# singhhp1069/charon

Measured on AMD Instinct MI355X. Metric: verified+aggregated 3-of-4 threshold BLS sigs/sec at 1/2/4/8 MI355X, higher is better.
Workload: dtype u32 (Fp 14x28-bit limbs); 1 GPU; config2: 3-of-4, 10000 DVs x 1 attestation per GPU; parallelism=shard1, inflight_launches=3, batches_per_launch=16, rlc_group=16, rlc_chunk=8, gident=0, subgroup_batch=0, level0=passed, hw_queues=4

## Files before the change

### charon_amd/csrc/bls_pair.h

```cpp
#pragma once
#include "bls_lines.h"

namespace tbg {

TBG_HD Fp pair_mul_lane(uint32_t par, const Fp& a, const Fp& ap, const Fp& b, const Fp& bp) {
  const Fp nbp = fp_neg_l(bp);
  return fp_mul2(a, fp_select(par != 0, bp, b), ap, fp_select(par != 0, b, nbp));
}
TBG_HD Fp pair_sqr_lane(uint32_t par, const Fp& a, const Fp& ap) {
  const Fp x = fp_add_l(fp_select(par != 0, ap, a), ap);
  const Fp y = fp_select(par != 0, a, fp_sub_l(a, ap));
  return fp_mul(x, y);
}
TBG_HD Fp pair_conj_lane(uint32_t par, const Fp& a) { return fp_select(par != 0, fp_neg(a), a); }
TBG_HD Fp pair_mul_xi_lane(uint32_t par, const Fp& a, const Fp& ap) {
  return fp_select(par != 0, fp_add(a, ap), fp_sub(a, ap));
}
TBG_HD Fp pair_inv_lane(uint32_t par, const Fp& a, const Fp& ap) {
  const Fp t = fp_inv(fp_mul2(a, a, ap, ap));
  return fp_mul(pair_conj_lane(par, a), t);
}
TBG_HD Fp pair_const(uint32_t par, const Fp2Const& c) { return par ? fp_from_const(c.c1) : fp_from_const(c.c0); }

struct Fp2p { Fp c0, c1; };
TBG_HD Fp2p f_add(const Fp2p& a, const Fp2p& b) { return {fp_add(a.c0, b.c0), fp_add(a.c1, b.c1)}; }
TBG_HD Fp2p f_sub(const Fp2p& a, const Fp2p& b) { return {fp_sub(a.c0, b.c0), fp_sub(a.c1, b.c1)}; }
TBG_HD Fp2p f_add_l(const Fp2p& a, const Fp2p& b) { return {fp_add_l(a.c0, b.c0), fp_add_l(a.c1, b.c1)}; }
TBG_HD Fp2p f_sub_l(const Fp2p& a, const Fp2p& b) { return {fp_sub_l(a.c0, b.c0), fp_sub_l(a.c1, b.c1)}; }
TBG_HD Fp2p f_neg(const Fp2p& a) { return {fp_neg(a.c0), fp_neg(a.c1)}; }
TBG_HD Fp2p f_reduce(const Fp2p& a) { return {fp_reduce(a.c0), fp_reduce(a.c1)}; }
TBG_HD Fp2p f_small(const Fp2p& a, uint32_t k) { return {fp_mul_small(a.c0, k), fp_mul_small(a.c1, k)}; }
TBG_HD Fp2p f_mul(const Fp2p& a, const Fp2p& b) {
  return {pair_mul_lane(0, a.c0, a.c1, b.c0, b.c1), pair_mul_lane(1, a.c1, a.c0, b.c1, b.c0)};
}
TBG_HD Fp2p f_sqr(const Fp2p& a) { return {pair_sqr_lane(0, a.c0, a.c1), pair_sqr_lane(1, a.c1, a.c0)}; }
TBG_HD Fp2p f_inv(const Fp2p& a) { return {pair_inv_lane(0, a.c0, a.c1), pair_inv_lane(1, a.c1, a.c0)}; }
TBG_HD bool f_is_zero(const Fp2p& a) { return fp_is_zero(a.c0) && fp_is_zero(a.c1); }
TBG_HD bool f_eq(const Fp2p& a, const Fp2p& b) { return fp_eq(a.c0, b.c0) && fp_eq(a.c1, b.c1); }
TBG_HD Fp2p pp_conj(const Fp2p& a) { return {pair_conj_lane(0, a.c0), pair_conj_lane(1, a.c1)}; }
TBG_HD Fp2p pp_mul_xi(const Fp2p& a) { return {pair_mul_xi_lane(0, a.c0, a.c1), pair_mul_xi_lane(1, a.c1, a.c0)}; }
TBG_HD Fp2p pp_mul_const(const Fp2p& a, const Fp2Const& c) {
  return {pair_mul_lane(0, a.c0, a.c1, pair_const(0, c), pair_const(1, c)),
          pair_mul_lane(1, a.c1, a.c0, pair_const(1, c), pair_const(0, c))};
}
TBG_HD Fp2p rlc_mul_c(const Fp2p& a, const Fp& c) { return {fp_mul(a.c0, c), fp_mul(a.c1, c)}; }
TBG_HD Fp2p f_conj(const Fp2p& a) { return pp_conj(a); }
TBG_HD Fp2p f_mulc(const Fp2p& a, const Fp2Const& c) { return pp_mul_const(a, c); }
template <> TBG_HD Fp2p f_zero<Fp2p>() { return {fp_zero(), fp_zero()}; }
template <> TBG_HD Fp2p f_one<Fp2p>() { return {fp_one(), fp_zero()}; }
TBG_HD Fp2p pp_from(const Fp2& a) { return {a.c0, a.c1}; }
TBG_HD Fp2 pp_to(const Fp2p& a) { return {a.c0, a.c1}; }

template <class F>
TBG_HD Jac<F> g2_psi_g(const Jac<F>& p) {
  return {f_mulc(f_conj(p.X), PSI_X), f_mulc(f_conj(p.Y), PSI_Y), f_reduce(f_conj(p.Z))};
}

template <class F>
TBG_HD Jac<F> jac_add_x(const Jac<F>& p, const Jac<F>& q, bool& exc) {
  if (jac_is_inf(p)) return q;
  if (jac_is_inf(q)) return p;
  const F Z1Z1 = f_sqr(p.Z);
  const F Z2Z2 = f_sqr(q.Z);
  const F S1 = f_mul(f_mul(p.Y, q.Z), Z2Z2);
  const F S2 = f_mul(f_mul(q.Y, p.Z), Z1Z1);
  const F Zs = f_reduce(f_sub_l(f_sqr(f_add(p.Z, q.Z)), f_add(Z1Z1, Z2Z2)));
  const F U1 = f_mul(p.X, Z2Z2);
  const F H = f_reduce(f_sub_l(f_mul(q.X, Z1Z1), U1));
  const F Rr = f_reduce(f_sub_l(S2, S1));
  if (f_is_zero(H)) {
    if (f_is_zero(Rr)) exc = true;
    return jac_inf<F>();
  }
  const F Z3 = f_mul(Zs, H);
  const F H2 = f_add(H, H);
  const F I = f_sqr(H2);
  const F J = f_mul(H, I);
  const F V = f_mul(U1, I);
  const F r2 = f_add(Rr, Rr);
  const F X3 = f_reduce(f_sub_l(f_sub_l(f_sqr(r2), J), f_add(V, V)));
  const F Y3 = f_reduce(f_sub_l(f_mul(f_sub_l(V, X3), r2), f_small(f_mul(S1, J), 2)));
  return {X3, Y3, Z3};
}

template <class F>
TBG_HD Jac<F> jac_dbl_lo(const Jac<F>& p) {
  const F YZ = f_mul(p.Y, p.Z);
  const F Z3 = f_reduce(f_add_l(YZ, YZ));
  const F B = f_sqr(p.Y);
  const F A = f_sqr(p.X);
  const F C = f_sqr(B);
  const F t = f_sub_l(f_sqr(f_add(p.X, B)), f_add(A, C));
  const F D = f_reduce(f_add_l(t, t));
  const F E = f_small(A, 3);
  const F X3 = f_reduce(f_sub_l(f_sqr(E), f_add(D, D)));
  const F Y3 = f_reduce(f_sub_l(f_mul(f_sub_l(D, X3), E), f_small(C, 8)));
  return {X3, Y3, Z3};
}

template <class F>
TBG_HD Jac<F> jac_add_aff_x(const Jac<F>& p, const Aff<F>& q, bool& exc) {
  if (jac_is_inf(p)) return jac_from_aff(q);
  F Z1Z1 = f_sqr(p.Z);
  F U2 = f_mul(q.x, Z1Z1);
  F S2 = f_mul(f_mul(q.y, p.Z), Z1Z1);
  F H = f_reduce(f_sub_l(U2, p.X));
  F Rr = f_reduce(f_sub_l(S2, p.Y));
  if (f_is_zero(H)) {
    if (f_is_zero(Rr)) exc = true;
    return jac_inf<F>();
  }
  F HH = f_sqr(H);
  F I = f_small(HH, 4);
  F J = f_mul(H, I);
  F r2 = f_add(Rr, Rr);
  F V = f_mul(p.X, I);
  F X3 = f_reduce(f_sub_l(f_sub_l(f_sqr(r2), J), f_add(V, V)));
  F Y3 = f_reduce(f_sub_l(f_mul(f_sub_l(V, X3), r2), f_small(f_mul(p.Y, J), 2)));
  F Z3 = f_reduce(f_sub_l(f_sub_l(f_sqr(f_add(p.Z, H)), Z1Z1), HH));
  return {X3, Y3, Z3};
}

template <class F>
TBG_HD Jac<F> jac_mul_xabs_aff_x(const Aff<F>& p, bool& exc) {
  Jac<F> acc = jac_from_aff(p);
#pragma unroll 1
  for (int i = 62; i >= 0; --i) {
    acc = jac_dbl_lo(acc);
    if ((X_ABS >> i) & 1) acc = jac_add_aff_x(acc, p, exc);
  }
  return acc;
}

template <class F>
TBG_HD Jac<F> jac_mul_xabs_x(const Jac<F>& p, bool& exc) {
  Jac<F> acc = p;
#pragma unroll 1
  for (int i = 62; i >= 0; --i) {
    acc = jac_dbl_lo(acc);
    if ((X_ABS >> i) & 1) acc = jac_add_x(acc, p, exc);
  }
  return acc;
}

template <class F>
TBG_HD Jac<F> g2_clear_cofactor_g(const Jac<F>& p, bool& exc) {
  const Jac<F> a = jac_neg(jac_mul_xabs_x(p, exc));
  const Jac<F> pp = g2_psi_g(p);
  const Jac<F> b = jac_add_x(a, pp, exc);
  Jac<F> u = g2_psi_g(g2_psi_g(jac_dbl_lo(p)));
  u = jac_add_x(u, jac_neg(pp), exc);
  u = jac_add_x(u, jac_neg(a), exc);
  u = jac_add_x(u, jac_neg(p), exc);
  const Jac<F> c = jac_neg(jac_mul_xabs_x(b, exc));
  return jac_add_x(u, c, exc);
}

template <class F> struct LineG { F l0, l1, l4; };

template <class F, bool EVAL = true, class S>
TBG_HD void miller_dbl_s(Jac<F>& T, const Fp& nxP, const Fp& yP, S&& sink) {
  const F ZZ = f_sqr(T.Z);
  const F YZ = f_mul(T.Y, T.Z);
  const F Z3 = f_reduce(f_add_l(YZ, YZ));
  const F l4 = f_mul(Z3, ZZ);
  sink(2, EVAL ? f_mulfp(l4, yP) : l4);
  const F B = f_sqr(T.Y);
  const F C = f_sqr(B);
  const F A = f_sqr(T.X);
  const F t = f_sub_l(f_sqr(f_add(T.X, B)), f_add(A, C));
  const F D = f_reduce(f_add_l(t, t));
  const F E = f_small(A, 3);
  const F l1 = f_mul(ZZ, E);
  sink(1, EVAL ? f_mulfp(l1, nxP) : l1);
  sink(0, f_reduce(f_sub_l(f_mul(T.X, E), f_add(B, B))));
  const F X3 = f_reduce(f_sub_l(f_sqr(E), f_add(D, D)));
  const F Y3 = f_reduce(f_sub_l(f_mul(f_sub_l(D, X3), E), f_small(C, 8)));
  T = {X3, Y3, Z3};
}

template <class F, bool EVAL = true, class S>
TBG_HD void miller_add_s(Jac<F>& T, const Aff<F>& Q, const Fp& nxP, const Fp& yP, S&& sink) {
  const F ZZ = f_sqr(T.Z);
  const F U2 = f_mul(Q.x, ZZ);
  const F S2 = f_mul(f_mul(Q.y, T.Z), ZZ);
  const F H = f_reduce(f_sub_l(U2, T.X));
  const F R = f_reduce(f_sub_l(S2, T.Y));
  const F Z3 = f_mul(T.Z, H);
  sink(2, EVAL ? f_mulfp(Z3, yP) : Z3);
  sink(1, EVAL ? f_mulfp(R, nxP) : R);
  sink(0, f_reduce(f_sub_l(f_mul(R, Q.x), f_mul(Q.y, Z3))));
  const F HH = f_sqr(H);
  const F HHH = f_mul(H, HH);
  const F V = f_mul(T.X, HH);
  const F X3 = f_reduce(f_sub_l(f_sub_l(f_sqr(R), HHH), f_add(V, V)));
  const F Y3 = f_reduce(f_sub_l(f_mul(f_sub_l(V, X3), R), f_mul(T.Y, HHH)));
  T = {X3, Y3, Z3};
}

template <class F, bool EVAL = true>
TBG_HD LineG<F> miller_dbl_g(Jac<F>& T, const Fp& nxP, const Fp& yP) {
  LineG<F> l;
  miller_dbl_s<F, EVAL>(T, nxP, yP, [&](int k, const F& v) { (k == 0 ? l.l0 : k == 1 ? l.l1 : l.l4) = v; });
  return l;
}

template <class F, bool EVAL = true>
TBG_HD LineG<F> miller_add_g(Jac<F>& T, const Aff<F>& Q, const Fp& nxP, const Fp& yP) {
// ... 122 lines not shown
```

### charon_amd/csrc/bls_rlc.h

```cpp
#pragma once
#include "bls_h2c.h"

namespace tbg {

TBG_HD void rlc_block(const uint32_t (&seed)[8], uint32_t i, uint32_t tag, uint32_t (&h)[8]) {
  uint32_t w[16];
#pragma unroll
  for (int k = 0; k < 8; ++k) w[k] = seed[k];
  w[8] = i;
  w[9] = tag;
#pragma unroll
  for (int k = 10; k < 16; ++k) w[k] = 0;
  sha256_iv(h);
  sha256_compress(h, w);
}
TBG_HD uint64_t rlc_scalar(const uint32_t (&seed)[8], uint32_t i) {
  uint32_t h[8];
  rlc_block(seed, i, 0x80000000u, h);
  uint64_t r = ((uint64_t)h[0] << 32) | h[1];
  return r ? r : 1;
}

TBG_HD void sgb_digits(const uint32_t (&seed)[8], uint32_t i, int32_t (&c)[18]) {
  uint8_t blk[64];
  for (int k = 0; k < 8; ++k) {
    blk[4 * k] = (uint8_t)(seed[k] >> 24);
    blk[4 * k + 1] = (uint8_t)(seed[k] >> 16);
    blk[4 * k + 2] = (uint8_t)(seed[k] >> 8);
    blk[4 * k + 3] = (uint8_t)seed[k];
  }
  for (int k = 32; k < 64; ++k) blk[k] = 0;
  blk[32] = (uint8_t)(i >> 24);
  blk[33] = (uint8_t)(i >> 16);
  blk[34] = (uint8_t)(i >> 8);
  blk[35] = (uint8_t)i;
  blk[36] = 0x53;
  blk[37] = 0x80;
  uint32_t h[8] = {0x6a09e667u, 0xbb67ae85u, 0x3c6ef372u, 0xa54ff53au, 0x510e527fu, 0x9b05688cu, 0x1f83d9abu, 0x5be0cd19u};
  sha256_block(h, blk);
  for (int k = 0; k < 18; ++k) {
    uint32_t w = h[k >> 2] % 28561u;
    for (int j = 0; j < (k & 3); ++j) w /= 13u;
    c[k] = (int32_t)(w % 13u) - 6;
  }
}

TBG_HD void rlc_digits(uint64_t r, uint32_t (&u)[4]) {
  for (int k = 0; k < 4; ++k) u[k] = (uint32_t)((r >> (16 * k)) & 0xFFFF);
}

TBG_HD G2A g2_psi_aff(const G2A& a) {
  return {fp2_mul(fp2_conj(a.x), fp2_from_const(PSI_X)), fp2_mul(fp2_conj(a.y), fp2_from_const(PSI_Y))};
}

TBG_HD Fp rlc_mul_c(const Fp& a, const Fp& c) { return fp_mul(a, c); }
TBG_HD Fp2 rlc_mul_c(const Fp2& a, const Fp& c) { return fp2_mul_fp(a, c); }

template <class F>
TBG_HD Aff<F> rlc_entry(const Aff<F>& ap, const Aff<F>& am, uint32_t b0, uint32_t b1, bool endo, const Fp& c) {
  const bool same = b0 == b1;
  const bool negy = (b0 != 0) == endo;
  Aff<F> e;
  e.x = same ? ap.x : am.x;
  const F y = same ? ap.y : am.y;
  const F ny = f_reduce(f_neg(y));
  e.y = negy ? ny : y;
  if (endo) e.x = rlc_mul_c(e.x, c);
  return e;
}

template <class F>
TBG_HD void rlc_pair_from_inv(const Aff<F>& q0, const Aff<F>& q1, const F& inv, Aff<F>& ap, Aff<F>& am) {
  const F lp = f_mul(f_reduce(f_sub(q1.y, q0.y)), inv);
  const F lm = f_mul(f_reduce(f_neg(f_reduce(f_add(q1.y, q0.y)))), inv);
  const F xs = f_reduce(f_add(q0.x, q1.x));
  ap.x = f_reduce(f_sub(f_sqr(lp), xs));
  ap.y = f_reduce(f_sub(f_mul(lp, f_reduce(f_sub(q0.x, ap.x))), q0.y));
  am.x = f_reduce(f_sub(f_sqr(lm), xs));
  am.y = f_reduce(f_sub(f_mul(lm, f_reduce(f_sub(q0.x, am.x))), q0.y));
}

template <class F>
TBG_HD Jac<F> rlc_mul_table(const Aff<F>& ap, const Aff<F>& am, const Fp& c, const uint32_t (&u)[4]) {
  Jac<F> acc = jac_from_aff(rlc_entry(ap, am, (u[0] >> 15) & 1, (u[1] >> 15) & 1, false, c));
  acc = jac_add_aff_in(acc, rlc_entry(ap, am, (u[2] >> 15) & 1, (u[3] >> 15) & 1, true, c));
#pragma unroll 1
  for (int bit = 14; bit >= 0; --bit) {
    acc = jac_dbl_in(acc);
    acc = jac_add_aff_in(acc, rlc_entry(ap, am, (u[0] >> bit) & 1, (u[1] >> bit) & 1, false, c));
    acc = jac_add_aff_in(acc, rlc_entry(ap, am, (u[2] >> bit) & 1, (u[3] >> bit) & 1, true, c));
  }
  return acc;
}

constexpr uint32_t PK_TAB_W2 = 8;
template <class F>
TBG_HD Jac<F> rlc_key_table_w2_entry(const Aff<F>& q0, const Aff<F>& q1, int k) {
  const int e0 = k >= 4 ? 3 : 1, e1 = 2 * (k & 3) - 3;
  const Jac<F> a = jac_from_aff(q0), b = jac_from_aff(q1);
  Jac<F> p0 = e0 == 3 ? jac_add(jac_dbl(a), a) : a;
  Jac<F> p1 = (e1 == 3 || e1 == -3) ? jac_add(jac_dbl(b), b) : b;
  if (e1 < 0) p1 = jac_neg(p1);
  return jac_add(p0, p1);
}
TBG_HD int rlc_win2(uint32_t u, int i) {
  return 2 * (2 * (int)((u >> (2 * i + 1)) & 1u) - 1) + (2 * (int)((u >> (2 * i)) & 1u) - 1);
}
template <class F>
TBG_HD Aff<F> rlc_entry_w2(const Aff<F>* tab, int v0, int v1, bool endo, const Fp& c) {
  const bool neg = v0 < 0;
  if (neg) {
    v0 = -v0;
    v1 = -v1;
  }
  Aff<F> e = tab[(v0 == 3 ? 4 : 0) + (v1 + 3) / 2];
  if (neg != endo) e.y = f_reduce(f_neg(e.y));
  if (endo) e.x = rlc_mul_c(e.x, c);
  return e;
}
template <class F>
TBG_HD Jac<F> rlc_mul_key_w2(const Aff<F>* tab, const Fp& c, const uint32_t (&u)[4]) {
  Jac<F> acc = jac_from_aff(rlc_entry_w2(tab, rlc_win2(u[0], 7), rlc_win2(u[1], 7), false, c));
  acc = jac_add_aff_in(acc, rlc_entry_w2(tab, rlc_win2(u[2], 7), rlc_win2(u[3], 7), true, c));
#pragma unroll 1
  for (int i = 6; i >= 0; --i) {
    acc = jac_dbl_in(jac_dbl_in(acc));
    acc = jac_add_aff_in(acc, rlc_entry_w2(tab, rlc_win2(u[0], i), rlc_win2(u[1], i), false, c));
    acc = jac_add_aff_in(acc, rlc_entry_w2(tab, rlc_win2(u[2], i), rlc_win2(u[3], i), true, c));
  }
  return acc;
}

#if defined(TBG_PK_W2)
TBG_HD G1J rlc_mul_key(const G1A* tab, const uint32_t (&u)[4]) {
#if TBG_PK_W2
  return rlc_mul_key_w2(tab, fp_from_const(G1_BETA), u);
#else
  return rlc_mul_table(tab[0], tab[1], fp_from_const(G1_BETA), u);
#endif
}
#endif

TBG_HD G2J rlc_mul_g2(const G2A& s, const uint32_t (&u)[4]) {
  const G2A ps = g2_psi_aff(s);
  G2A ap, am;
  rlc_pair_from_inv(s, ps, fp2_inv(fp2_reduce(fp2_sub(ps.x, s.x))), ap, am);
  return rlc_mul_table(ap, am, fp_from_const(PSI2_X), u);
}

TBG_HD G1J rlc_mul_g1(const G1A& pk, const G1A& xpk, const uint32_t (&u)[4]) {
  G1A ap, am;
  rlc_pair_from_inv(pk, xpk, fp_inv(fp_reduce(fp_sub(xpk.x, pk.x))), ap, am);
  return rlc_mul_table(ap, am, fp_from_const(G1_BETA), u);
}

TBG_HD void rlc_mul_both(const G2A& s, const G1A& pk, const G1A& xpk, const uint32_t (&u)[4], G2J& S, G1J& P) {
  const G2A ps = g2_psi_aff(s);
  const Fp2 dx2 = fp2_reduce(fp2_sub(ps.x, s.x));
  const Fp dx1 = fp_reduce(fp_sub(xpk.x, pk.x));
  const Fp n2 = fp_mul2(dx2.c0, dx2.c0, dx2.c1, dx2.c1);
  const Fp t = fp_inv(fp_mul(n2, dx1));
  const Fp in2 = fp_mul(t, dx1);
  {
    G2A ap, am;
    rlc_pair_from_inv(s, ps, Fp2{fp_mul(dx2.c0, in2), fp_mul(fp_neg(dx2.c1), in2)}, ap, am);
    S = rlc_mul_table(ap, am, fp_from_const(PSI2_X), u);
  }
  {
    G1A ap, am;
    rlc_pair_from_inv(pk, xpk, fp_mul(t, n2), ap, am);
    P = rlc_mul_table(ap, am, fp_from_const(G1_BETA), u);
  }
}

template <class F>
TBG_HD Jac<F> rlc_entry_j(const Jac<F>& ap, const Jac<F>& am, uint32_t b0, uint32_t b1, bool endo, const Fp& c) {
  const bool same = b0 == b1;
  const bool negy = (b0 != 0) == endo;
  Jac<F> e;
  e.X = same ? ap.X : am.X;
  e.Z = same ? ap.Z : am.Z;
  const F y = same ? ap.Y : am.Y;
  const F ny = f_reduce(f_neg(y));
  e.Y = negy ? ny : y;
  if (endo) e.X = rlc_mul_c(e.X, c);
  return e;
}

template <class F>
TBG_HD void rlc_pair_jac(const Aff<F>& q0, const Aff<F>& q1, Jac<F>& ap, Jac<F>& am) {
  const Jac<F> j0 = jac_from_aff(q0);
  ap = jac_add_aff_in(j0, q1);
  am = jac_add_aff_in(j0, Aff<F>{q1.x, f_reduce(f_neg(q1.y))});
}

template <class F>
TBG_HD Jac<F> rlc_mul_table_j(const Jac<F>& ap, const Jac<F>& am, const Fp& c, const uint32_t (&u)[4]) {
  Jac<F> acc = rlc_entry_j(ap, am, (u[0] >> 15) & 1, (u[1] >> 15) & 1, false, c);
  acc = jac_add_in<F, true>(acc, rlc_entry_j(ap, am, (u[2] >> 15) & 1, (u[3] >> 15) & 1, true, c));
#pragma unroll 1
  for (int bit = 14; bit >= 0; --bit) {
    acc = jac_dbl_in(acc);
    acc = jac_add_in<F, true>(acc, rlc_entry_j(ap, am, (u[0] >> bit) & 1, (u[1] >> bit) & 1, false, c));
    acc = jac_add_in<F, true>(acc, rlc_entry_j(ap, am, (u[2] >> bit) & 1, (u[3] >> bit) & 1, true, c));
  }
  return acc;
}

TBG_HD G1J rlc_mul_g1_j(const G1A& pk, const G1A& xpk, const uint32_t (&u)[4]) {
  G1J ap, am;
  rlc_pair_jac(pk, xpk, ap, am);
  return rlc_mul_table_j(ap, am, fp_from_const(G1_BETA), u);
}

}
```

### charon_amd/csrc/k_decode.hip

```cpp
#define TBG_ADD_DBL_INLINE 1
#ifndef TBG_SCHED_FENCE
#define TBG_SCHED_FENCE 1
#endif
#include "tbls_launch.h"
#include "bls_curve.h"
#include "bls_pair.h"
#include "bls_batchinv.h"

namespace tbg {

__global__ void __launch_bounds__(BINV_BLOCK) k_decode_pubkeys(const uint8_t* pk48, uint32_t n, G1A* out, G1A* out_x,
                                                               int32_t* status) {
  const uint32_t i = blockIdx.x * blockDim.x + threadIdx.x;
  const bool in = i < n;
  G1A a{fp_zero(), fp_zero()}, ax = a;
  int32_t st = DEC_ERR_FLAGS;
  G1J xa = jac_inf<Fp>();
  if (in) {
    uint8_t b[48];
    for (int j = 0; j < 48; ++j) b[j] = pk48[48ull * i + j];
    st = g1_decompress(b, a);
    if (st == DEC_OK) xa = jac_neg(jac_mul_xabs(jac_from_aff(a)));
  }
  const bool ok = block_jac_to_aff<BINV_WAVES>(xa, in && st == DEC_OK, ax);
  if (!in) return;
  if (st != DEC_OK || !ok) {
    if (st == DEC_OK) st = DEC_IDENTITY;
    a.x = fp_zero();
    a.y = fp_zero();
    ax = a;
  }
  out[i] = a;
  out_x[i] = ax;
  status[i] = st;
}

__global__ void TBG_LAUNCH_N(TBG_DECODE_WAVES) k_decode_sigs(DevBatch B) {
  uint32_t i = blockIdx.x * blockDim.x + threadIdx.x;
  if (i < CNT_WORDS) B.counters[i] = 0;
  if (B.rlc_batch && i <= MSM_BUCKETS) B.msm_off[i] = 0;
  if (i >= B.n_partials) return;
  G2A& a = B.sig_aff[i];
  int32_t st = g2_decompress_t<true, false>(B.sigs + 96ull * i, a, SlotKeep{&a.y});
  if (st == DEC_IDENTITY) st = TBG_PS_ERR_IDENTITY;
  if (st != DEC_OK) {
    a.x = fp2_zero();
    a.y = fp2_zero();
  }
  B.partial_status[i] = (st == DEC_OK) ? TBG_PS_NOT_VERIFIED : st;
}

__global__ void TBG_LAUNCH_N(TBG_PAIR_WAVES) k_subgroup_sigs(DevBatch B) {
  const uint32_t i = (blockIdx.x * blockDim.x + threadIdx.x) >> 1;
  if (i >= B.n_partials) return;
  if (B.partial_status[i] != TBG_PS_NOT_VERIFIED) return;
  if (B.sgb && !B.sgb_bad[i / B.sgb_m]) return;
  const Aff<Fp2x> a = px_load(B.sig_aff[i]);
  bool exc = false;
  bool ok = g2_in_subgroup_aff_g(a, exc);
  if (exc) {
    ok = g2_in_subgroup(jac_from_aff(B.sig_aff[i]));
  }
  if (!ok && pair_par() == 0) {
    B.partial_status[i] = TBG_PS_ERR_SUBGROUP;
    B.sig_aff[i] = G2A{fp2_zero(), fp2_zero()};
  }
}

void launch_decode_pubkeys(const uint8_t* pk48, uint32_t n, G1A* out, G1A* out_x, int32_t* status, hipStream_t st) {
  if (n) TBG_KLAUNCH(k_decode_pubkeys, dim3((n + BINV_BLOCK - 1) / BINV_BLOCK), dim3(BINV_BLOCK), st, pk48, n, out,
                     out_x, status);
}
void launch_decode_sigs(const DevBatch& B, hipStream_t st) {
  uint32_t lanes = B.n_partials > CNT_WORDS ? B.n_partials : CNT_WORDS;
  if (B.rlc_batch && lanes < MSM_BUCKETS + 1) lanes = MSM_BUCKETS + 1;
  TBG_KLAUNCH(k_decode_sigs, grid_for(lanes), dim3(kBlock), st, B);
  launch_subgroup_batch(B, st);
  if (B.n_partials) TBG_KLAUNCH(k_subgroup_sigs, grid_for(2 * B.n_partials), dim3(kBlock), st, B);
}

}
```

### charon_amd/csrc/k_gmsm.hip

```cpp
#define TBG_ADD_DBL_INLINE 1
#ifndef TBG_SCHED_FENCE
#define TBG_SCHED_FENCE 1
#endif
#include "tbls_launch.h"
#include "bls_msm.h"
#include "bls_pair.h"

namespace tbg {

constexpr uint32_t kGmSortBlock = 64;
constexpr uint32_t kGmMaxBlocks = 2048;

inline dim3 gm_grid(uint64_t threads, uint32_t block) {
  const uint64_t b = (threads + block - 1) / block;
  return dim3((uint32_t)(b < kGmMaxBlocks ? (b ? b : 1) : kGmMaxBlocks));
}

__device__ __forceinline__ uint32_t gm_groups(const DevBatch& B) { return (B.n_duties + B.rlc_group - 1) / B.rlc_group; }

__device__ __forceinline__ bool gm_member(const DevBatch& B, uint32_t i) {
  return B.partial_status[i] == TBG_PS_NOT_VERIFIED && B.dv_state[B.partial_duty[i]] == RLC_COMBINED;
}

__global__ void TBG_LAUNCH k_rlc_g1(DevBatch B, const G1A* tab, const G1A* pk_aff, const int32_t* pk_status,
                                   uint32_t n_pk) {
  const uint32_t i = blockIdx.x * blockDim.x + threadIdx.x;
  if (i >= B.n_partials || B.partial_status[i] != TBG_PS_NOT_VERIFIED) return;
  const uint32_t pid = B.pubkey_ids[i];
  if (pid >= n_pk || pk_status[pid] != DEC_OK) {
    B.partial_status[i] = TBG_PS_ERR_PUBKEY;
    return;
  }
  const uint32_t d = B.partial_duty[i];
  const uint32_t d0 = (d / B.rlc_group) * B.rlc_group;
  bool lead = true;
  for (uint32_t j = B.duty_first[d0]; j < i && lead; ++j) {
    const int32_t st = B.partial_status[j];
    const uint32_t q = B.pubkey_ids[j];
    lead = !((st == TBG_PS_NOT_VERIFIED || st == TBG_PS_ERR_PUBKEY) && q < n_pk && pk_status[q] == DEC_OK);
  }
  if (lead) {
    B.part_p[i] = jac_from_aff(pk_aff[pid]);
    return;
  }
  uint32_t u[4];
  rlc_digits(rlc_scalar(B.rlc_seed, i), u);
  B.part_p[i] = rlc_mul_key(tab + (size_t)PK_TAB * pid, u);
}

__global__ void __launch_bounds__(kGmSortBlock) k_gm_sort(DevBatch B) {
  if (B.counters[CNT_L0_OK]) return;
  __shared__ uint32_t cnt[GM_BUCKETS];
  __shared__ uint32_t lead;
  const uint32_t t = threadIdx.x, G = B.rlc_group, ng = gm_groups(B);
#pragma unroll 1
  for (uint32_t g = blockIdx.x; g < ng; g += gridDim.x) {
    const uint32_t d0 = g * G, d1 = min(d0 + G, B.n_duties);
    const uint32_t p0 = B.duty_first[d0], p1 = B.duty_first[d1];
    if (t < GM_BUCKETS) cnt[t] = 0;
    if (t == 0) lead = 0xFFFFFFFFu;
    if (g == blockIdx.x)
      for (uint32_t k = t; k < 256u && blockIdx.x == 0; k += kGmSortBlock) B.gm_hist[k] = 0;
    __syncthreads();
    if (!B.rlc_batch)
      for (uint32_t i = p0 + t; i < p1; i += kGmSortBlock)
        if (B.partial_status[i] == TBG_PS_NOT_VERIFIED) atomicMin(&lead, i);
    __syncthreads();
    const uint32_t ld = lead;
    for (uint32_t i = p0 + t; i < p1; i += kGmSortBlock) {
      if (!gm_member(B, i)) continue;
      if (i == ld) {
        atomicAdd(&cnt[0], 1u);
        continue;
      }
      uint32_t u[4];
      rlc_digits(rlc_scalar(B.rlc_seed, i), u);
#pragma unroll
      for (uint32_t k = 0; k < 4; ++k)
#pragma unroll
        for (uint32_t w = 0; w < GM_W; ++w) {
          bool neg;
          atomicAdd(&cnt[gm_bucket(u[k], w, neg)], 1u);
        }
    }
    __syncthreads();
    uint32_t* off = B.gm_off + (size_t)(GM_BUCKETS + 1) * g;
    if (t == 0) {
      uint32_t run = 0;
      for (uint32_t b = 0; b < GM_BUCKETS; ++b) {
        const uint32_t c = cnt[b];
        off[b] = run;
        cnt[b] = run;
        run += c;
      }
      off[GM_BUCKETS] = run;
      B.gm_lead[g] = ld;
    }
    __syncthreads();
    uint32_t* ent = B.gm_ent + 16ull * p0;
    for (uint32_t i = p0 + t; i < p1; i += kGmSortBlock) {
      if (!gm_member(B, i)) continue;
      if (i == ld) {
        ent[atomicAdd(&cnt[0], 1u)] = msm_entry(i, 0, false);
        continue;
      }
      uint32_t u[4];
      rlc_digits(rlc_scalar(B.rlc_seed, i), u);
#pragma unroll 1
      for (uint32_t k = 0; k < 4; ++k)
#pragma unroll
        for (uint32_t w = 0; w < GM_W; ++w) {
          bool neg;
          const uint32_t b = gm_bucket(u[k], w, neg);
          ent[atomicAdd(&cnt[b], 1u)] = msm_entry(i, k, neg);
        }
    }
    __syncthreads();
  }
}

__device__ __forceinline__ Aff<Fp2x> gm_point(const G2A& s, uint32_t k, bool neg) {
  Aff<Fp2x> p = px_load(s);
  p.y = f_reduce(p.y);
  if (k & 1) p = Aff<Fp2x>{f_mulc(f_conj(p.x), PSI_X), f_mulc(f_conj(p.y), PSI_Y)};
  const bool ny = ((k & 2) != 0) != neg;
  if (k & 2) p.x = f_mulfp(p.x, fp_from_const(PSI2_X));
  if (ny) p.y = f_reduce(f_neg(p.y));
  return p;
}

constexpr uint32_t GM_SIZES = 256;
__global__ void TBG_LAUNCH k_gm_hist(DevBatch B) {
  if (B.counters[CNT_L0_OK]) return;
  __shared__ uint32_t h[GM_SIZES];
  for (uint32_t k = threadIdx.x; k < GM_SIZES; k += blockDim.x) h[k] = 0;
  __syncthreads();
  const uint32_t n = gm_groups(B) * GM_BUCKETS;
  for (uint32_t x = blockIdx.x * blockDim.x + threadIdx.x; x < n; x += gridDim.x * blockDim.x) {
    const uint32_t* off = B.gm_off + (size_t)(GM_BUCKETS + 1) * (x / GM_BUCKETS) + x % GM_BUCKETS;
    atomicAdd(&h[min(off[1] - off[0], GM_SIZES - 1)], 1u);
  }
  __syncthreads();
  for (uint32_t k = threadIdx.x; k < GM_SIZES; k += blockDim.x)
    if (h[k]) atomicAdd(&B.gm_hist[k], h[k]);
}
__global__ void __launch_bounds__(64) k_gm_hist_scan(DevBatch B) {
  if (B.counters[CNT_L0_OK] || threadIdx.x) return;
  uint32_t run = 0;
  for (int k = (int)GM_SIZES - 1; k >= 0; --k) {
    const uint32_t c = B.gm_hist[k];
    B.gm_hist[k] = run;
    run += c;
  }
}
__global__ void TBG_LAUNCH k_gm_order(DevBatch B) {
  if (B.counters[CNT_L0_OK]) return;
  __shared__ uint32_t h[GM_SIZES];
  const uint32_t n = gm_groups(B) * GM_BUCKETS;
  const uint32_t per = (n + gridDim.x - 1) / gridDim.x;
  const uint32_t x0 = min(n, blockIdx.x * per), x1 = min(n, x0 + per);
  for (uint32_t k = threadIdx.x; k < GM_SIZES; k += blockDim.x) h[k] = 0;
  __syncthreads();
  auto cls = [&](uint32_t x) {
    const uint32_t* off = B.gm_off + (size_t)(GM_BUCKETS + 1) * (x / GM_BUCKETS) + x % GM_BUCKETS;
    return min(off[1] - off[0], GM_SIZES - 1);
  };
  for (uint32_t x = x0 + threadIdx.x; x < x1; x += blockDim.x) atomicAdd(&h[cls(x)], 1u);
  __syncthreads();
  for (uint32_t k = threadIdx.x; k < GM_SIZES; k += blockDim.x)
    if (h[k]) h[k] = atomicAdd(&B.gm_hist[k], h[k]);
  __syncthreads();
  for (uint32_t x = x0 + threadIdx.x; x < x1; x += blockDim.x) B.gm_order[atomicAdd(&h[cls(x)], 1u)] = x;
}

__global__ void TBG_LAUNCH_N(TBG_PAIR_WAVES) k_gm_bucket(DevBatch B) {
  if (B.counters[CNT_L0_OK]) return;
  const uint32_t n = gm_groups(B) * GM_BUCKETS;
  const uint32_t stride = (gridDim.x * blockDim.x) >> 1;
// ... 102 lines not shown
```

### charon_amd/csrc/k_miller_hex.hip

```cpp
#ifndef TBG_SCHED_FENCE
#define TBG_SCHED_FENCE 1
#endif
#include "tbls_launch.h"
#include "bls_lines.h"
#include "bls_hex.h"

namespace tbg {

#ifndef TBG_HEX_HOIST
#define TBG_HEX_HOIST 1
#endif
constexpr uint32_t HEX_HOIST_MAX = 16;

#ifndef TBG_HEX_PREFETCH
#define TBG_HEX_PREFETCH 0
#endif

#if TBG_HEX_PREFETCH
struct HexSqrMask { uint64_t lo, hi; };
constexpr HexSqrMask hex_sqr_mask() {
  HexSqrMask m{0, 0};
  int idx = 0;
  for (int b = 62; b >= 0; --b) {
    if (b != 62) {
      if (idx < 64) m.lo |= 1ull << idx;
      else m.hi |= 1ull << (idx - 64);
    }
    idx += ((X_ABS >> b) & 1) ? 2 : 1;
  }
  return m;
}
constexpr HexSqrMask kHexSqr = hex_sqr_mask();
static_assert(N_LINES <= 128, "line mask");

constexpr uint32_t HEX_PF_WORDS = 64 * NL;
__shared__ uint32_t s_pf_a[HEX_PF_WORDS];
__shared__ uint32_t s_pf_b[HEX_PF_WORDS];

template <int BUF>
TBG_DEV void hex_pf_issue(const uint32_t* h_lines, uint32_t m, int idx, uint32_t after = 0) {
  uint32_t* buf = BUF ? s_pf_b : s_pf_a;
  const uint32_t k = 2u * (uint32_t)quad_lane() + hex_c();
  uint32_t z = 0;
  asm volatile("" : "+v"(z) : "v"(after));
  const uint32_t* src = h_lines + (size_t)LINES_WORDS * m + LINE_WORDS * idx + k * NL + z;
#pragma unroll
  for (int i = 0; i < NL; ++i)
    __builtin_amdgcn_global_load_lds((const void*)(src + i), (__attribute__((address_space(3))) void*)(buf + 64 * i), 4,
                                     0, 0);
}
template <int BUF>
TBG_DEV Fp hex_pf_read(uint32_t L) {
  const uint32_t* buf = BUF ? s_pf_b : s_pf_a;
  Fp r;
#pragma unroll
  for (int i = 0; i < NL; ++i) r.l[i] = buf[64 * i + L];
  return r;
}

template <int BUF>
TBG_DEV Fp4h hex_pf_step(const Fp4h& A, const DevBatch& B, uint32_t d, uint32_t nm, int nidx) {
  const uint32_t c = hex_c();
  const int q = quad_lane();
  const uint32_t lane = threadIdx.x & 63u;
  const uint32_t base = (lane & ~16u) - (uint32_t)q;
  const Fp nv = hex_line_operand(B.dv_p[d]);
  const Fp lk = hex_pf_read<BUF>(base + (q == 0 ? 1u : 2u) + (c << 4));
  const Fp e = fp_mul(lk, nv);
  hex_pf_issue<BUF ^ 1>(B.h_lines, nm, nidx < 0 ? N_LINES - 1 : nidx, e.l[0]);
  const Fp e1 = xch<QP_B0>(e), e4 = xch<QP_B1>(e);
  HxLine r;
  {
    const Fp4h An = hxch<QP_NEXT>(A);
    hx_line_u(c, hx_own_par(An, hx_swap(An)), Fp2o{e1, hx_swap(e1)}, r);
  }
  const Fp2o l0{hex_pf_read<BUF>(base + (c << 4)), hex_pf_read<BUF>(base + ((c ^ 1u) << 4))};
  hx_line_t(c, q, hx_own_par(A, hx_swap(A)), l0, Fp2o{e4, hx_swap(e4)}, r);
  return hx_line2(c, q, r, hx_swap(r.W));
}

TBG_DEV Fp4h hex_chunk_staged(const DevBatch& B, uint32_t d0, uint32_t run, const uint32_t* my_msg) {
  Fp4h f = hex_one();
  if (!run) return f;
  uint32_t bits = run;
  int idx = 0;
  uint32_t j = __builtin_ctz(bits);
  hex_pf_issue<0>(B.h_lines, my_msg[j], 0);
  auto advance = [&](uint32_t& nj, int& nidx) {
    const uint32_t rest = bits & (bits - 1);
    if (rest) {
      nj = __builtin_ctz(rest);
      nidx = idx;
    } else {
      nj = __builtin_ctz(run);
      nidx = idx + 1 < N_LINES ? idx + 1 : -1;
    }
  };
  auto sqr_before = [](int i) {
    return i < 64 ? ((kHexSqr.lo >> i) & 1u) != 0 : ((kHexSqr.hi >> (i - 64)) & 1u) != 0;
  };
#pragma unroll 1
  for (;;) {
    uint32_t nj;
    int nidx;
    if (bits == run && sqr_before(idx)) f = hex_sqr(f);
    advance(nj, nidx);
    f = hex_pf_step<0>(f, B, d0 + j, my_msg[nj], nidx);
    if (nidx < 0) break;
    bits = bits & (bits - 1);
    if (!bits) bits = run;
    idx = nidx;
    j = nj;
    if (bits == run && sqr_before(idx)) f = hex_sqr(f);
    advance(nj, nidx);
    f = hex_pf_step<1>(f, B, d0 + j, my_msg[nj], nidx);
    if (nidx < 0) break;
    bits = bits & (bits - 1);
    if (!bits) bits = run;
    idx = nidx;
    j = nj;
  }
  asm volatile("s_waitcnt vmcnt(0)" ::: "memory");
  return f;
}
#endif

template <int MODE>
__global__ void TBG_LAUNCH_N(TBG_HEX_WAVES) k_miller_hex(DevBatch B) {
  const uint32_t t = blockIdx.x * blockDim.x + threadIdx.x;
  const uint32_t G = B.rlc_group, C = B.rlc_chunk;
  const uint32_t n_groups = (B.n_duties + G - 1) / G;
  const uint32_t nch = (G + C - 1) / C, nq = nch + 1;
  const uint32_t np_q = MODE == MILLER_GROUP_S ? 0u : n_groups * nch;
  const uint32_t qd = hex_slot(t);
  if (qd == 0xFFFFFFFFu || qd >= np_q + (MODE == MILLER_L0 ? 1u : n_groups)) return;
  if (MODE == MILLER_GROUP_S && B.counters[CNT_L0_OK]) return;
  const bool s_quad = qd >= np_q;
  const uint32_t* ls = nullptr;
  uint32_t* dst;
  uint32_t d0 = 0, d1 = 0;
  if (MODE == MILLER_L0 && s_quad) {
    if (B.counters[CNT_L0_BAD]) return;
    ls = B.batch_lines;
    dst = B.batch_f;
  } else {
    const uint32_t g = s_quad ? qd - np_q : qd / nch, c = s_quad ? nch : qd % nch;
    if (MODE != MILLER_L0) {
      const int32_t gs = B.grp_state[g];
      if (gs == GRP_EMPTY || (gs == GRP_FAIL && s_quad)) return;
    }
    if (s_quad) {
      ls = B.grp_lines + (size_t)LINES_WORDS * g;
    } else {
      d0 = g * G + c * C;
      d1 = min(d0 + C, min(g * G + G, B.n_duties));
    }
    dst = B.chunk_f + (size_t)3 * 4 * NL * (g * nq + c);
  }
  Fp4h f = hex_one();
  int idx = 0;
#if TBG_HEX_HOIST
  __shared__ uint32_t s_msg[kBlock * HEX_HOIST_MAX];
  uint32_t* my_msg = s_msg + HEX_HOIST_MAX * threadIdx.x;
  const bool hoist = d1 - d0 <= HEX_HOIST_MAX;
  uint32_t run = 0;
  if (hoist) {
    for (uint32_t d = d0; d < d1; ++d) {
      if (B.dv_state[d] != RLC_COMBINED) continue;
      const uint32_t m = B.duty_msg[d];
      if (B.h_status[m] != 0) continue;
      my_msg[d - d0] = m;
      run |= 1u << (d - d0);
    }
  }
#if TBG_HEX_PREFETCH
  if (hoist && !s_quad) {
    hex_store(dst, hex_chunk_staged(B, d0, run, my_msg));
    return;
  }
#endif
#endif
#pragma unroll 1
  for (int b = 62; b >= 0; --b) {
    if (b != 62) f = hex_sqr(f);
    const int steps = ((X_ABS >> b) & 1) ? 2 : 1;
#pragma unroll 1
    for (int s = 0; s < steps; ++s, ++idx) {
      if (s_quad) f = hex_line_folded(f, ls, idx);
#if TBG_HEX_HOIST
      if (hoist) {
#pragma unroll 1
        for (uint32_t bits = run; bits; bits &= bits - 1) {
          const uint32_t j = __builtin_ctz(bits);
          f = hex_line_at_v(f, B.h_lines + (size_t)LINES_WORDS * my_msg[j], idx, hex_line_operand(B.dv_p[d0 + j]));
        }
        continue;
      }
#endif
#pragma unroll 1
      for (uint32_t d = d0; d < d1; ++d) {
        if (B.dv_state[d] != RLC_COMBINED) continue;
        const uint32_t m = B.duty_msg[d];
        if (B.h_status[m] != 0) continue;
        f = hex_line_at_v(f, B.h_lines + (size_t)LINES_WORDS * m, idx, hex_line_operand(B.dv_p[d]));
      }
    }
  }
  hex_store(dst, f);
}

void launch_l0_miller_hex(const DevBatch& B, hipStream_t st) {
  const uint32_t n_groups = (B.n_duties + B.rlc_group - 1) / B.rlc_group;
  const uint32_t nch = (B.rlc_group + B.rlc_chunk - 1) / B.rlc_chunk;
  TBG_KLAUNCH(k_miller_hex<MILLER_L0>, grid_for(hex_threads(n_groups * nch + 1)), dim3(kBlock), st, B);
}
void launch_groups_miller_hex(const DevBatch& B, hipStream_t st) {
  const uint32_t n_groups = (B.n_duties + B.rlc_group - 1) / B.rlc_group;
  const uint32_t nch = (B.rlc_group + B.rlc_chunk - 1) / B.rlc_chunk;
  TBG_KLAUNCH(k_miller_hex<MILLER_GROUPS>, grid_for(hex_threads(n_groups * (nch + 1))), dim3(kBlock), st, B);
}
void launch_group_s_miller_hex(const DevBatch& B, hipStream_t st) {
  const uint32_t n_groups = (B.n_duties + B.rlc_group - 1) / B.rlc_group;
  TBG_KLAUNCH(k_miller_hex<MILLER_GROUP_S>, grid_for(hex_threads(n_groups)), dim3(kBlock), st, B);
}

}
```

### charon_amd/csrc/k_msm.hip

```cpp
#define TBG_ADD_DBL_INLINE 1
#ifndef TBG_SCHED_FENCE
#define TBG_SCHED_FENCE 1
#endif
#include "tbls_launch.h"
#include "bls_msm.h"
#include "bls_pair.h"
#include "bls_batchinv.h"

namespace tbg {

__global__ void __launch_bounds__(BINV_BLOCK) k_pubkey_tables(const G1A* pk, const G1A* xpk, const int32_t* status,
                                                              uint32_t n, G1A* tab) {
  const uint32_t i = blockIdx.x * blockDim.x + threadIdx.x;
  const bool in = i < n;
  const bool ok = in && status[i] == DEC_OK;
  G1A p0{fp_zero(), fp_zero()}, x0 = p0;
  if (ok) {
    p0 = pk[i];
    x0 = xpk[i];
  }
#if TBG_PK_W2
#pragma unroll 1
  for (int k = 0; k < (int)PK_TAB; ++k) {
    const G1J e = ok ? rlc_key_table_w2_entry(p0, x0, k) : jac_inf<Fp>();
    G1A a{fp_zero(), fp_zero()};
    const bool got = block_jac_to_aff<BINV_WAVES>(e, ok, a);
    if (in) tab[(size_t)PK_TAB * i + k] = got ? a : G1A{fp_zero(), fp_zero()};
  }
#else
  const Fp t = block_batch_inv<BINV_WAVES>(fp_reduce(fp_sub(x0.x, p0.x)), ok);
  if (!in) return;
  G1A ap{fp_zero(), fp_zero()}, am = ap;
  if (ok) rlc_pair_from_inv(p0, x0, t, ap, am);
  tab[2ull * i] = ap;
  tab[2ull * i + 1] = am;
#endif
}

__global__ void TBG_LAUNCH k_rlc_g1_l0(DevBatch B, const G1A* tab, const int32_t* pk_status, uint32_t n_pk) {
  const uint32_t i = blockIdx.x * blockDim.x + threadIdx.x;
  if (i >= B.n_partials || B.partial_status[i] != TBG_PS_NOT_VERIFIED) return;
  const uint32_t pid = B.pubkey_ids[i];
  if (pid >= n_pk || pk_status[pid] != DEC_OK) {
    B.partial_status[i] = TBG_PS_ERR_PUBKEY;
    return;
  }
  const uint64_t r = rlc_scalar(B.rlc_seed, i);
  uint32_t u[4];
  rlc_digits(r, u);
  B.msm_r[i] = r;
  B.part_p[i] = rlc_mul_key(tab + (size_t)PK_TAB * pid, u);
#pragma unroll
  for (int k = 0; k < 4; ++k) {
    bool neg;
    atomicAdd(&B.msm_off[msm_bucket(u[k], neg)], 1u);
  }
}

constexpr int kScanBlock = 1024;
__global__ void __launch_bounds__(kScanBlock) k_msm_scan(DevBatch B) {
  TBG_URGENT();
  __shared__ uint32_t part[kScanBlock];
  constexpr uint32_t per = MSM_BUCKETS / kScanBlock;
  const uint32_t t = threadIdx.x, j0 = t * per;
  uint32_t sum = 0;
  for (uint32_t j = 0; j < per; ++j) sum += B.msm_off[j0 + j];
  part[t] = sum;
  __syncthreads();
  for (uint32_t d = 1; d < kScanBlock; d <<= 1) {
    const uint32_t v = t >= d ? part[t - d] : 0u;
    __syncthreads();
    part[t] += v;
    __syncthreads();
  }
  uint32_t run = part[t] - sum;
  for (uint32_t j = 0; j < per; ++j) {
    const uint32_t c = B.msm_off[j0 + j];
    B.msm_off[j0 + j] = run;
    B.msm_cur[j0 + j] = run;
    run += c;
  }
  if (t == kScanBlock - 1) B.msm_off[MSM_BUCKETS] = run;
}

__global__ void TBG_LAUNCH k_msm_scatter(DevBatch B) {
  const uint32_t i = blockIdx.x * blockDim.x + threadIdx.x;
  if (i >= B.n_partials || B.partial_status[i] != TBG_PS_NOT_VERIFIED) return;
  uint32_t u[4];
  rlc_digits(B.msm_r[i], u);
#pragma unroll
  for (uint32_t k = 0; k < 4; ++k) {
    bool neg;
    const uint32_t j = msm_bucket(u[k], neg);
    B.msm_ent[atomicAdd(&B.msm_cur[j], 1u)] = msm_entry(i, k, neg);
  }
}

__device__ __forceinline__ Aff<Fp2x> px_psi_k(const G2A& s, uint32_t k, bool neg) {
  Aff<Fp2x> p = px_load(s);
  p.y = f_reduce(p.y);
  if (k & 1) p = Aff<Fp2x>{f_mulc(f_conj(p.x), PSI_X), f_mulc(f_conj(p.y), PSI_Y)};
  const bool ny = ((k & 2) != 0) != neg;
  if (k & 2) p.x = f_mulfp(p.x, fp_from_const(PSI2_X));
  if (ny) p.y = f_reduce(f_neg(p.y));
  return p;
}

__global__ void TBG_LAUNCH_N(TBG_PAIR_WAVES) k_msm_bucket_part(DevBatch B) {
  const uint32_t w = (blockIdx.x * blockDim.x + threadIdx.x) >> 1;
  if (w >= MSM_BUCKETS * MSM_SPLIT) return;
  if (B.counters[CNT_L0_BAD]) return;
  const uint32_t j = w / MSM_SPLIT, sl = w % MSM_SPLIT;
  const uint32_t o0 = B.msm_off[j], n = B.msm_off[j + 1] - o0;
  const uint32_t e0 = o0 + (n * sl) / MSM_SPLIT, e1 = o0 + (n * (sl + 1)) / MSM_SPLIT;
  Jac<Fp2x> acc = jac_inf<Fp2x>();
#pragma unroll 1
  for (uint32_t e = e0; e < e1; ++e) {
    const uint32_t v = B.msm_ent[e];
    acc = jac_add_aff_in(acc, px_psi_k(B.sig_aff[v >> 3], (v >> 1) & 3u, (v & 1u) != 0));
  }
  px_store(B.msm_part[w], acc);
}

template <bool FAST>
__device__ __forceinline__ Jac<Fp2x> msm_bucket_scaled(const DevBatch& B, uint32_t j, bool& exc) {
  Jac<Fp2x> acc = px_load(B.msm_part[MSM_SPLIT * j]);
#pragma unroll 1
  for (uint32_t sl = 1; sl < MSM_SPLIT; ++sl) {
    const Jac<Fp2x> q = px_load(B.msm_part[MSM_SPLIT * j + sl]);
    acc = FAST ? jac_add_x(acc, q, exc) : jac_add(acc, q);
  }
  const uint32_t m = 2 * j + 1;
  if (m > 1 && !jac_is_inf(acc)) {
    px_store(B.msm_bkt[j], acc);
    const int top = 31 - __builtin_clz(m);
#pragma unroll 1
    for (int bit = top - 1; bit >= 0; --bit) {
      acc = jac_dbl_in(acc);
      if ((m >> bit) & 1u) {
        __asm__ __volatile__("" ::: "memory");
        const Jac<Fp2x> b = px_load(B.msm_bkt[j]);
        acc = FAST ? jac_add_x(acc, b, exc) : jac_add(acc, b);
      }
    }
  }
  return acc;
}
#ifndef TBG_MSM_BUCKET_X
#define TBG_MSM_BUCKET_X 1
#endif
__device__ __noinline__ Jac<Fp2x> msm_bucket_complete(const DevBatch& B, uint32_t j) {
  bool unused = false;
  return msm_bucket_scaled<false>(B, j, unused);
}

__global__ void TBG_LAUNCH_N(TBG_PAIR_WAVES) k_msm_bucket(DevBatch B) {
  TBG_URGENT();
  const uint32_t j = (blockIdx.x * blockDim.x + threadIdx.x) >> 1;
  if (j >= MSM_BUCKETS) return;
  if (B.counters[CNT_L0_BAD]) return;
#if TBG_MSM_BUCKET_X
  bool exc = false;
  Jac<Fp2x> acc = msm_bucket_scaled<true>(B, j, exc);
  if (!pair_all(!exc)) acc = msm_bucket_complete(B, j);
#else
  Jac<Fp2x> acc = px_load(B.msm_part[MSM_SPLIT * j]);
#pragma unroll 1
  for (uint32_t sl = 1; sl < MSM_SPLIT; ++sl) acc = jac_add_in<Fp2x, true>(acc, px_load(B.msm_part[MSM_SPLIT * j + sl]));
  const uint32_t m = 2 * j + 1;
  if (m > 1 && !jac_is_inf(acc)) {
    const Jac<Fp2x> b = acc;
    const int top = 31 - __builtin_clz(m);
#pragma unroll 1
    for (int bit = top - 1; bit >= 0; --bit) {
      acc = jac_dbl_in(acc);
      if ((m >> bit) & 1u) acc = jac_add_in<Fp2x, true>(acc, b);
    }
  }
#endif
  px_store(B.msm_bkt[j], acc);
}

constexpr uint32_t MSM_TREE_PAIRS = 128;
constexpr uint32_t MSM_TREE_PER = 4;
constexpr uint32_t MSM_TREE_WG = MSM_BUCKETS / (MSM_TREE_PAIRS * MSM_TREE_PER);
static_assert(MSM_TREE_WG <= 2 * 64 && MSM_TREE_WG <= MSM_SUM_ENTRIES, "second tree kernel: one workgroup");

template <uint32_t PAIRS>
__device__ __forceinline__ Jac<Fp2x> pair_tree_sum(Jac<Fp2x> acc, Jac<Fp2x>* lds) {
  const uint32_t t = threadIdx.x, pr = t >> 1;
#pragma unroll 1
  for (uint32_t s = 1; s < PAIRS; s <<= 1) {
    lds[t] = acc;
    __syncthreads();
    if ((pr & (2 * s - 1)) == 0 && pr + s < PAIRS) acc = jac_add_in<Fp2x, true>(acc, lds[t + 2 * s]);
    __syncthreads();
  }
  return acc;
}

__global__ void __launch_bounds__(2 * MSM_TREE_PAIRS) k_msm_tree(DevBatch B) {
  TBG_URGENT();
  __shared__ Jac<Fp2x> lds[2 * MSM_TREE_PAIRS];
  if (B.counters[CNT_L0_BAD]) return;
  const uint32_t pr = threadIdx.x >> 1;
  const uint32_t a0 = (blockIdx.x * MSM_TREE_PAIRS + pr) * MSM_TREE_PER;
  Jac<Fp2x> acc = px_load(B.msm_bkt[a0]);
#pragma unroll 1
  for (uint32_t a = a0 + 1; a < a0 + MSM_TREE_PER; ++a) acc = jac_add_in<Fp2x, true>(acc, px_load(B.msm_bkt[a]));
  acc = pair_tree_sum<MSM_TREE_PAIRS>(acc, lds);
  if (pr == 0) px_store(B.msm_sum[blockIdx.x], acc);
}

__global__ void __launch_bounds__(MSM_TREE_WG) k_msm_tree_final(DevBatch B) {
  TBG_URGENT();
  constexpr uint32_t PAIRS = MSM_TREE_WG / 2;
  __shared__ Jac<Fp2x> lds[2 * PAIRS];
  if (B.counters[CNT_L0_BAD]) return;
  const uint32_t pr = threadIdx.x >> 1;
  Jac<Fp2x> acc = jac_add_in<Fp2x, true>(px_load(B.msm_sum[2 * pr]), px_load(B.msm_sum[2 * pr + 1]));
  acc = pair_tree_sum<PAIRS>(acc, lds);
  if (pr != 0) return;
  if (jac_is_inf(acc)) {
    if (pair_par() == 0) B.counters[CNT_L0_BAD] = 1;
    return;
  }
  const Fp2x zi = f_inv(acc.Z);
  const Fp2x zi2 = f_sqr(zi);
  px_store(*B.batch_pt, Aff<Fp2x>{f_mul(acc.X, zi2), f_mul(acc.Y, f_mul(zi2, zi))});
}

void launch_pubkey_tables(const G1A* pk, const G1A* xpk, const int32_t* status, uint32_t n, G1A* tab, hipStream_t st) {
  if (n) TBG_KLAUNCH(k_pubkey_tables, dim3((n + BINV_BLOCK - 1) / BINV_BLOCK), dim3(BINV_BLOCK), st, pk, xpk, status, n,
                     tab);
}

void launch_l0_keys(const DevBatch& B, const G1A* pk_tab, const int32_t* pk_status, uint32_t n_pk, hipStream_t st) {
  if (B.n_partials) TBG_KLAUNCH(k_rlc_g1_l0, grid_for(B.n_partials), dim3(kBlock), st, B, pk_tab, pk_status, n_pk);
}

void launch_l0_msm(const DevBatch& B, hipStream_t st) {
  TBG_KLAUNCH(k_msm_scan, dim3(1), dim3(kScanBlock), st, B);
  if (B.n_partials) TBG_KLAUNCH(k_msm_scatter, grid_for(B.n_partials), dim3(kBlock), st, B);
  TBG_KLAUNCH(k_msm_bucket_part, grid_for(2 * MSM_BUCKETS * MSM_SPLIT), dim3(kBlock), st, B);
  TBG_KLAUNCH(k_msm_bucket, grid_for(2 * MSM_BUCKETS), dim3(kBlock), st, B);
  TBG_KLAUNCH(k_msm_tree, dim3(MSM_TREE_WG), dim3(2 * MSM_TREE_PAIRS), st, B);
  TBG_KLAUNCH(k_msm_tree_final, dim3(1), dim3(MSM_TREE_WG), st, B);
}

}
```

### charon_amd/csrc/k_rlc.hip

```cpp
#define TBG_ADD_DBL_INLINE 1
#ifndef TBG_SCHED_FENCE
#define TBG_SCHED_FENCE 1
#endif
#include "tbls_launch.h"
#include "bls_h2c.h"
#include "bls_lines.h"
#include "bls_hex.h"
#include "bls_rlc.h"
#include "bls_batchinv.h"
#include "bls_row.h"

namespace tbg {

__device__ __forceinline__ bool rlc_usable(const DevBatch& B, uint32_t i, const int32_t* pk_status, uint32_t n_pk) {
  int32_t st = B.partial_status[i];
  if (st != TBG_PS_NOT_VERIFIED && st != TBG_PS_ERR_PUBKEY) return false;
  uint32_t pid = B.pubkey_ids[i];
  return pid < n_pk && pk_status[pid] == DEC_OK;
}
__device__ __forceinline__ bool rlc_candidate(const DevBatch& B, uint32_t i) {
  return B.partial_status[i] == TBG_PS_NOT_VERIFIED;
}

__device__ __forceinline__ bool rlc_combinable(const DevBatch& B, uint32_t d) {
  return B.dv_state[d] == RLC_COMBINED && B.h_status[B.duty_msg[d]] == 0;
}
__device__ __forceinline__ uint32_t rlc_candidates(const DevBatch& B, uint32_t d) {
  uint32_t n = 0;
  for (uint32_t i = B.duty_first[d]; i < B.duty_first[d + 1]; ++i) n += rlc_candidate(B, i) ? 1u : 0u;
  return n;
}


template <int PHASE>
__global__ void __launch_bounds__(BINV_BLOCK) k_rlc_duty_sum(DevBatch B) {
  constexpr int phase = PHASE;
  const uint32_t d = blockIdx.x * blockDim.x + threadIdx.x;
  const bool in = d < B.n_duties;
  if (phase == DSUM_FALLBACK_S) {
    if (!in || B.counters[CNT_L0_OK] || B.dv_state[d] != RLC_COMBINED) return;
#if TBG_GMSM
    const int32_t gs = B.grp_state[d / B.rlc_group];
    if (gs != GRP_FAIL && gs != GRP_GID) return;
#endif
    G2J S = jac_inf<Fp2>();
    for (uint32_t i = B.duty_first[d]; i < B.duty_first[d + 1]; ++i)
      if (rlc_candidate(B, i)) S = jac_add(S, B.part_s[i]);
    B.dv_s[d] = S;
    return;
  }
  G1J P = jac_inf<Fp>();
  G2J S = jac_inf<Fp2>();
  int cand = 0;
  if (in) {
    for (uint32_t i = B.duty_first[d]; i < B.duty_first[d + 1]; ++i) {
      if (!rlc_candidate(B, i)) continue;
      P = jac_add_in<Fp, true>(P, B.part_p[i]);
      if (phase == DSUM_BOTH) S = jac_add(S, B.part_s[i]);
      ++cand;
    }
  }
  G1A Pa;
  const bool aff = block_jac_to_aff<BINV_WAVES>(P, cand > 0, Pa);
  if (!in) return;
  if (cand == 0) {
    B.dv_state[d] = RLC_NONE;
    return;
  }
  if (!aff || (phase == DSUM_BOTH && jac_is_inf(S))) {
    B.dv_state[d] = RLC_EACH;
    if (phase == DSUM_L0_P) B.counters[CNT_L0_BAD] = 1;
    return;
  }
  B.dv_p[d] = G1A{fp_reduce(fp_neg(Pa.x)), Pa.y};
  if (phase == DSUM_BOTH) B.dv_s[d] = S;
  B.dv_state[d] = RLC_COMBINED;
}
inline dim3 duty_grid(const DevBatch& B) { return dim3((B.n_duties + BINV_BLOCK - 1) / BINV_BLOCK); }

__global__ void TBG_LAUNCH k_rlc_group_lines(DevBatch B) {
  if (B.counters[CNT_L0_OK]) return;
  uint32_t g = blockIdx.x * blockDim.x + threadIdx.x;
  uint32_t G = B.rlc_group;
  uint32_t n_groups = (B.n_duties + G - 1) / G;
  if (g >= n_groups) return;
  uint32_t d0 = g * G, d1 = min(d0 + G, B.n_duties);
  G2J S = jac_inf<Fp2>();
  int n = 0;
  for (uint32_t d = d0; d < d1; ++d)
    if (B.dv_state[d] == RLC_COMBINED) {
      S = jac_add(S, B.dv_s[d]);
      ++n;
    }
  G2A Sa;
  if (n == 0) {
    B.grp_state[g] = GRP_EMPTY;
    return;
  }
  if (!jac_to_aff(S, Sa)) {
    B.grp_state[g] = GRP_FAIL;
    return;
  }
  B.pend_pts[g] = Sa;
  B.grp_state[g] = GRP_LINES;
}

constexpr int QUAD_WORDS = 4 * NL;


__global__ void TBG_LAUNCH_N(TBG_HEX_WAVES) k_rlc_group_final(DevBatch B) {
  uint32_t t = blockIdx.x * blockDim.x + threadIdx.x;
  uint32_t G = B.rlc_group, C = B.rlc_chunk;
  uint32_t n_groups = (B.n_duties + G - 1) / G;
  uint32_t nq = (G + C - 1) / C + 1;
  uint32_t g = hex_slot(t);
  if (g >= n_groups) return;
  const bool lead = hex_lead();
  if (B.grp_state[g] != GRP_LINES) return;
  uint32_t d0 = g * G, d1 = min(d0 + G, B.n_duties);
  for (uint32_t d = d0; d < d1; ++d) {
    if (B.dv_state[d] == RLC_COMBINED && B.h_status[B.duty_msg[d]] != 0) {
      if (lead) B.grp_state[g] = GRP_FAIL;
      return;
    }
  }
  const uint32_t* base = B.chunk_f + (size_t)3 * QUAD_WORDS * nq * g;
  Fp4h f = hex_load(base);
  for (uint32_t c = 1; c < nq; ++c) f = hex_mul_ni(f, hex_load(base + (size_t)3 * QUAD_WORDS * c));
  f = hex_final_exp_in(hex_conj(f));
  bool ok = hex_is_one(f);
  if (!ok && B.gident) {
    uint32_t m = 0;
    for (uint32_t d = d0; d < d1; ++d)
      if (rlc_combinable(B, d)) m += rlc_candidates(B, d);
    if (m >= 2) {
      uint32_t slot = 0;
      if (lead) slot = atomicAdd(&B.counters[CNT_GID], 1u);
      slot = (uint32_t)__shfl((int)slot, (int)hex_lead_lane());
      hex_store(B.grp_fe + (size_t)3 * QUAD_WORDS * slot, f);
      if (lead) {
        B.gid_list[slot] = g;
        B.grp_state[g] = GRP_GID;
      }
      return;
    }
  }
  if (lead) B.grp_state[g] = ok ? GRP_OK : GRP_FAIL;
}

__global__ void TBG_LAUNCH_N(TBG_HEX_WAVES) k_l0_fold(DevBatch B) {
  TBG_URGENT();
  const uint32_t t = blockIdx.x * blockDim.x + threadIdx.x;
  const uint32_t G = B.rlc_group, C = B.rlc_chunk;
  const uint32_t n_groups = (B.n_duties + G - 1) / G, nch = (G + C - 1) / C, nq = nch + 1;
  const uint32_t g = hex_slot(t);
  if (g >= n_groups || B.counters[CNT_L0_BAD]) return;
  const uint32_t d0 = g * G, d1 = min(d0 + G, B.n_duties);
  for (uint32_t d = d0; d < d1; ++d) {
    if (B.dv_state[d] == RLC_COMBINED && B.h_status[B.duty_msg[d]] != 0) {
      if (hex_lead()) B.counters[CNT_L0_BAD] = 1;
      return;
    }
  }
  const uint32_t* base = B.chunk_f + (size_t)3 * QUAD_WORDS * nq * g;
  Fp4h f = hex_load(base);
  for (uint32_t c = 1; c < nch; ++c) f = hex_mul(f, hex_load(base + (size_t)3 * QUAD_WORDS * c));
  hex_store(B.grp_f + (size_t)3 * QUAD_WORDS * g, f);
}

__global__ void TBG_LAUNCH_N(TBG_HEX_WAVES) k_l0_tree(DevBatch B, uint32_t in, uint32_t n, uint32_t out) {
  TBG_URGENT();
  const uint32_t t = blockIdx.x * blockDim.x + threadIdx.x;
  const uint32_t q = hex_slot(t);
  if (q == 0xFFFFFFFFu || q * L0_TREE_FAN >= n || B.counters[CNT_L0_BAD]) return;
  const uint32_t a0 = q * L0_TREE_FAN, a1 = min(a0 + L0_TREE_FAN, n);
  Fp4h f = hex_load(B.grp_f + (size_t)3 * QUAD_WORDS * (in + a0));
  for (uint32_t a = a0 + 1; a < a1; ++a) f = hex_mul(f, hex_load(B.grp_f + (size_t)3 * QUAD_WORDS * (in + a)));
  hex_store(B.grp_f + (size_t)3 * QUAD_WORDS * (out + q), f);
}

constexpr uint32_t L0_FINAL_THREADS = 16 * 36;
__device__ __forceinline__ int32_t* l0_f_spare(const DevBatch& B, int k) {
  const uint32_t n_groups = (B.n_duties + B.rlc_group - 1) / B.rlc_group;
  return (int32_t*)(B.grp_f + (size_t)3 * QUAD_WORDS * (grp_f_entries(n_groups) - 1 - k));
}
__global__ void __launch_bounds__(L0_FINAL_THREADS) k_l0_final(DevBatch B, uint32_t in, uint32_t n) {
  TBG_URGENT();
  if (B.counters[CNT_L0_BAD]) return;
  __shared__ RowSlots S;
  RowDevExec ex;
  const int r = threadIdx.x >> 4, j = threadIdx.x & 15;
// ... 390 lines not shown

__device__ __forceinline__ void push_group_chunks(const DevBatch& B, uint32_t g) {
  const uint32_t G = B.rlc_group, C = B.rlc_chunk, nch = (G + C - 1) / C;
  for (uint32_t c = 0; c < nch; ++c) {
    const uint32_t dc0 = g * G + c * C, dc1 = min(min(dc0 + C, g * G + G), B.n_duties);
    for (uint32_t d = dc0; d < dc1; ++d)
      if (rlc_combinable(B, d)) {
        B.chunk_list[atomicAdd(&B.counters[CNT_CHUNKS], 1u)] = g * nch + c;
        break;
      }
  }
}

__global__ void TBG_LAUNCH_N(TBG_HEX_WAVES) k_rlc_gident_miller(DevBatch B) {
  const uint32_t t = blockIdx.x * blockDim.x + threadIdx.x;
  const uint32_t G = B.rlc_group, C = B.rlc_chunk, nch = (G + C - 1) / C, nq = nch + 1;
  const uint32_t s = hex_slot(t);
  if (s == 0xFFFFFFFFu) return;
  const uint32_t k = s / nq + B.fb_base, c = s % nq;
  if (k >= B.counters[CNT_GID] || !fb_in_pass(B, k)) return;
  const uint32_t entry = B.gid_list[k];
  if (entry & ID_DEGENERATE) return;
  const uint32_t g = entry, gd0 = g * G, gd1 = min(gd0 + G, B.n_duties);
  const uint32_t d0 = c == nch ? gd0 : min(gd0 + c * C, gd1), d1 = c == nch ? gd0 : min(d0 + C, gd1);
  const uint32_t* ls = B.gid_lines + fb_slot(B, k);
  const G1A* wp = B.gid_p + (size_t)G * k;
  const Fp4h f = hex_miller([&](Fp4h x, int idx) {
    if (c == nch) x = hex_line_folded(x, ls, idx);
#pragma unroll 1
    for (uint32_t d = d0; d < d1; ++d) {
      if (!rlc_combinable(B, d)) continue;
      const G1A& P = wp[d - gd0];
      x = hex_line_at(x, B.h_lines + (size_t)LINES_WORDS * B.duty_msg[d], idx, P.x, P.y);
    }
    return x;
  });
  hex_store(B.gid_f + (size_t)3 * QUAD_WORDS * ((size_t)k * nq + c), f);
}

#ifndef TBG_GID_L3_MAX
#define TBG_GID_L3_MAX 40u
#endif

__global__ void TBG_LAUNCH_N(TBG_HEX_WAVES) k_rlc_gident_check(DevBatch B) {
  const uint32_t t = blockIdx.x * blockDim.x + threadIdx.x;
  const uint32_t k = hex_slot(t) + B.fb_base;
  if (hex_slot(t) == 0xFFFFFFFFu || k >= B.counters[CNT_GID] || !fb_in_pass(B, k)) return;
  const bool lead = hex_lead();
  const uint32_t G = B.rlc_group, C = B.rlc_chunk, nq = (G + C - 1) / C + 1;
  const uint32_t entry = B.gid_list[k], g = entry & ~ID_DEGENERATE;
  const uint32_t d0 = g * G, d1 = min(d0 + G, B.n_duties);
  uint32_t found = 0, m = 0;
  for (uint32_t d = d0; d < d1; ++d)
    if (rlc_combinable(B, d)) m += rlc_candidates(B, d);
  if (!(entry & ID_DEGENERATE)) {
    const uint32_t* base = B.gid_f + (size_t)3 * QUAD_WORDS * ((size_t)k * nq);
    Fp4h f = hex_load(base);
    for (uint32_t c = 1; c < nq; ++c) f = hex_mul_ni(f, hex_load(base + (size_t)3 * QUAD_WORDS * c));
    const Fp4h inv_a2 = hex_final_exp_in(f);
    found = hex_find_power(hex_load(B.grp_fe + (size_t)3 * QUAD_WORDS * k), inv_a2, m);
  }
  if (!lead) return;
  if (!found) {
    if (B.gident == 2 || m > TBG_GID_L3_MAX) {
      push_group_chunks(B, g);
    } else {
      for (uint32_t d = d0; d < d1; ++d)
        if (rlc_combinable(B, d)) rlc_push_partials(B, d);
    }
    return;
  }
  uint32_t w = 0;
  for (uint32_t d = d0; d < d1; ++d) {
    if (!rlc_combinable(B, d)) continue;
    for (uint32_t i = B.duty_first[d]; i < B.duty_first[d + 1]; ++i) {
      if (!rlc_candidate(B, i)) continue;
      B.partial_status[i] = ++w == found ? TBG_PS_INVALID : TBG_PS_VALID;
    }
  }
}

__global__ void TBG_LAUNCH k_list_all_partials(DevBatch B, const int32_t* pk_status, uint32_t n_pk) {
  uint32_t i = blockIdx.x * blockDim.x + threadIdx.x;
  if (i >= B.n_partials) return;
  if (!rlc_candidate(B, i)) return;
  uint32_t pid = B.pubkey_ids[i];
  if (pid >= n_pk || pk_status[pid] != DEC_OK) {
    B.partial_status[i] = TBG_PS_ERR_PUBKEY;
    return;
  }
  B.part_list[atomicAdd(&B.counters[CNT_PARTIALS], 1u)] = i;
}

__global__ void TBG_LAUNCH_N(TBG_PAIR_WAVES) k_lines_sig_list(DevBatch B) {
  fb_pass_loop(B, (blockIdx.x * blockDim.x + threadIdx.x) >> 1, (gridDim.x * blockDim.x) >> 1,
               B.counters[CNT_PARTIALS], [&](uint32_t k) {
    const uint32_t i = B.part_list[k];
    const Fp nx = fp_reduce(fp_neg(fp_from_const(G1_X)));
    Aff<Fp2x> q = px_load(B.sig_aff[i]);
    q = {f_reduce(q.x), f_reduce(q.y)};
    px_g2_lines(q, nx, fp_from_const(G1_NEG_Y), B.sig_lines + fb_slot(B, k));
  });
}

TBG_DEV uint32_t hex_grid_slots() { return gridDim.x * (blockDim.x / 64u) * 10u; }

__global__ void TBG_LAUNCH_N(TBG_HEX_WAVES) k_verify_list(DevBatch B, const G1A* pk_aff) {
  const uint32_t t = blockIdx.x * blockDim.x + threadIdx.x;
  if (hex_slot(t) == 0xFFFFFFFFu) return;
  const bool lead = hex_lead();
  fb_pass_loop(B, hex_slot(t), hex_grid_slots(), B.counters[CNT_PARTIALS], [&](uint32_t k) {
    uint32_t i = B.part_list[k];
    uint32_t m = B.duty_msg[B.partial_duty[i]];
    if (B.h_status[m] != 0) {
      if (lead) B.partial_status[i] = TBG_PS_INVALID;
      return;
    }
    G1A pk = pk_aff[B.pubkey_ids[i]];
    Fp nx = fp_reduce(fp_neg(pk.x));
    const uint32_t* ls = B.sig_lines + fb_slot(B, k);
    const uint32_t* lh = B.h_lines + (size_t)LINES_WORDS * m;
    Fp4h f = hex_miller([&](Fp4h x, int idx) { return hex_line_at(hex_line_folded(x, ls, idx), lh, idx, nx, pk.y); });
    f = hex_final_exp_in(hex_conj(f));
    const bool ok = hex_is_one(f);
    if (lead) B.partial_status[i] = ok ? TBG_PS_VALID : TBG_PS_INVALID;
  });
}

constexpr uint32_t FB_SMALL = 640;
template <class F>
static void fb_passes(const DevBatch& B, uint32_t max_entries, F&& body, bool may_shrink = false) {
  const uint32_t W = B.fb_window ? B.fb_window : max_entries;
  for (uint32_t base = 0; base < max_entries; base += W) {
    DevBatch P = B;
    P.fb_base = base;
    const uint32_t n = max_entries - base < W ? max_entries - base : W;
    body(P, may_shrink && base > 0 && base >= B.fb_full && n > FB_SMALL ? FB_SMALL : n);
  }
}

void launch_rlc_prepare(const DevBatch& B, const G1A* pk_aff, const G1A* xpk_aff, const G1A* pk_tab,
                        const int32_t* pk_status, uint32_t n_pk, hipStream_t st,
                        void (*after_keys)(const DevBatch&, hipStream_t)) {
  if (!B.n_duties) return;
  if (B.rlc_group == 0) {
    if (B.n_partials) TBG_KLAUNCH(k_list_all_partials, grid_for(B.n_partials), dim3(kBlock), st, B, pk_status, n_pk);
    if (after_keys) after_keys(B, st);
    return;
  }
  uint32_t n_groups = (B.n_duties + B.rlc_group - 1) / B.rlc_group;
  if (B.rlc_batch) {
    launch_l0_keys(B, pk_tab, pk_status, n_pk, st);
    if (after_keys) after_keys(B, st);
    launch_l0_msm(B, st);
    TBG_KLAUNCH(k_rlc_duty_sum<DSUM_L0_P>, duty_grid(B), dim3(BINV_BLOCK), st, B);
    launch_l0_lines(B, st);
    return;
  }
  if (after_keys) after_keys(B, st);
#if TBG_GMSM
  launch_rlc_g1(B, pk_tab, pk_aff, pk_status, n_pk, st);
  TBG_KLAUNCH(k_rlc_duty_sum<DSUM_P>, duty_grid(B), dim3(BINV_BLOCK), st, B);
  launch_gm_group_s(B, st);
#else
  launch_rlc_partials(B, pk_tab, pk_aff, pk_status, n_pk, st);
  TBG_KLAUNCH(k_rlc_duty_sum<DSUM_BOTH>, duty_grid(B), dim3(BINV_BLOCK), st, B);
  TBG_KLAUNCH(k_rlc_group_lines, grid_for(n_groups), dim3(kBlock), st, B);
#endif
  launch_lines_fold(B, FOLD_GROUPS, n_groups, st);
}

void launch_rlc_check(const DevBatch& B, const G1A* pk_aff, const G1A* xpk_aff, const int32_t* pk_status, uint32_t n_pk,
                      hipStream_t st) {
  if (!B.n_duties) return;
  if (B.rlc_group != 0) {
    uint32_t n_groups = (B.n_duties + B.rlc_group - 1) / B.rlc_group;
    uint32_t nch = (B.rlc_group + B.rlc_chunk - 1) / B.rlc_chunk;
    if (B.rlc_batch) {
      launch_l0_miller_hex(B, st);
      TBG_KLAUNCH(k_l0_fold, grid_for(hex_threads(n_groups)), dim3(kBlock), st, B);
      uint32_t in = 0, n = n_groups, out = n_groups;
      while (n > L0_TREE_FAN) {
        const uint32_t m = (n + L0_TREE_FAN - 1) / L0_TREE_FAN;
        TBG_KLAUNCH(k_l0_tree, grid_for(hex_threads(m)), dim3(kBlock), st, B, in, n, out);
        in = out;
        out += m;
        n = m;
      }
      launch_l0_final(B, in, n, st);
      TBG_KLAUNCH(k_l0_after, grid_for(n_groups), dim3(kBlock), st, B);
#if TBG_GMSM
      launch_gm_group_s(B, st);
#else
      launch_rlc_partials(B, nullptr, pk_aff, pk_status, n_pk, st);
      TBG_KLAUNCH(k_rlc_duty_sum<DSUM_FALLBACK_S>, duty_grid(B), dim3(BINV_BLOCK), st, B);
      TBG_KLAUNCH(k_rlc_group_lines, grid_for(n_groups), dim3(kBlock), st, B);
#endif
      launch_lines_fold(B, FOLD_GROUPS, n_groups, st);
      launch_group_s_miller_hex(B, st);
    } else {
      launch_groups_miller_hex(B, st);
    }
    TBG_KLAUNCH(k_rlc_group_final, grid_for(hex_threads(n_groups)), dim3(kBlock), st, B);
    TBG_KLAUNCH(k_rlc_resolve_groups, grid_for(B.n_duties), dim3(kBlock), st, B);
#if TBG_GMSM
    launch_gm_failed_partials(B, pk_aff, st);
    TBG_KLAUNCH(k_rlc_duty_sum<DSUM_FALLBACK_S>, duty_grid(B), dim3(BINV_BLOCK), st, B);
#endif
    if (B.rlc_group > 1) {
      uint32_t W = 1;
      while (W < B.rlc_group) W <<= 1;
      TBG_KLAUNCH(k_rlc_gident_lines, grid_for(n_groups * W), dim3(kBlock), st, B);
      fb_passes(B, n_groups, [&](const DevBatch& P, uint32_t n) {
        launch_lines_fold(P, FOLD_GID, n, st);
        TBG_KLAUNCH(k_rlc_gident_miller, grid_for(hex_threads(n * (nch + 1))), dim3(kBlock), st, P);
        TBG_KLAUNCH(k_rlc_gident_check, grid_for(hex_threads(n)), dim3(kBlock), st, P);
      });
      TBG_KLAUNCH(k_rlc_chunk_lines, grid_for(n_groups * nch), dim3(kBlock), st, B);
      fb_passes(B, n_groups * nch, [&](const DevBatch& P, uint32_t n) {
        launch_lines_fold(P, FOLD_CHUNKS, n, st);
        TBG_KLAUNCH(k_rlc_check_chunks, grid_for(hex_threads(n)), dim3(kBlock), st, P);
      });
      TBG_KLAUNCH(k_rlc_cident_lines, grid_for(n_groups * nch), dim3(kBlock), st, B);
      fb_passes(B, n_groups * nch, [&](const DevBatch& P, uint32_t n) {
        launch_lines_fold(P, FOLD_CID, n, st);
        TBG_KLAUNCH(k_rlc_cident_check, grid_for(hex_threads(n)), dim3(kBlock), st, P);
      });
      TBG_KLAUNCH(k_rlc_ident_lines, grid_for(B.n_duties), dim3(kBlock), st, B);
      fb_passes(B, B.n_duties, [&](const DevBatch& P, uint32_t n) {
        launch_lines_fold(P, FOLD_IDENT, n, st);
        TBG_KLAUNCH(k_rlc_ident_check, grid_for(hex_threads(n)), dim3(kBlock), st, P);
      }, true);
    }
  }
  if (B.n_partials) {
    fb_passes(B, B.n_partials, [&](const DevBatch& P, uint32_t n) {
      TBG_KLAUNCH(k_lines_sig_list, grid_for(2 * n), dim3(kBlock), st, P);
      TBG_KLAUNCH(k_verify_list, grid_for(hex_threads(n)), dim3(kBlock), st, P, pk_aff);
    }, true);
  }
}

}
```

### charon_amd/csrc/k_sgb.hip

```cpp
#define TBG_ADD_DBL_INLINE 1
#ifndef TBG_SCHED_FENCE
#define TBG_SCHED_FENCE 1
#endif
#include "tbls_launch.h"
#include "bls_rlc.h"
#include "bls_pair.h"

namespace tbg {

#ifndef TBG_SGB_SORT_BLOCK
#define TBG_SGB_SORT_BLOCK 256
#endif
constexpr uint32_t kSgbSortBlock = TBG_SGB_SORT_BLOCK;

__global__ void __launch_bounds__(kSgbSortBlock) k_sgb_sort(DevBatch B) {
  __shared__ uint32_t cnt[SGB_BUCKETS];
  __shared__ uint32_t off[SGB_BUCKETS + 1];
  __shared__ int8_t dig[SGB_M * SGB_K];
  const uint32_t g = blockIdx.x, t = threadIdx.x, m = B.sgb_m;
  const uint32_t i0 = g * m;
  const uint32_t n = min(m, B.n_partials - i0);
  for (uint32_t b = t; b < SGB_BUCKETS; b += kSgbSortBlock) cnt[b] = 0;
  if (t == 0) B.sgb_bad[g] = 0;
  __syncthreads();
  for (uint32_t li = t; li < n; li += kSgbSortBlock) {
    const bool ok = B.partial_status[i0 + li] == TBG_PS_NOT_VERIFIED;
    int32_t c[SGB_K];
    sgb_digits(B.sgb_seed, i0 + li, c);
#pragma unroll
    for (uint32_t k = 0; k < SGB_K; ++k) {
      const int32_t d = ok ? c[k] : 0;
      dig[li * SGB_K + k] = (int8_t)d;
      if (d) atomicAdd(&cnt[k * SGB_V + (uint32_t)(d < 0 ? -d : d) - 1], 1u);
    }
  }
  __syncthreads();
  if (t == 0) {
    uint32_t run = 0;
    for (uint32_t b = 0; b < SGB_BUCKETS; ++b) {
      off[b] = run;
      run += cnt[b];
    }
    off[SGB_BUCKETS] = run;
  }
  __syncthreads();
  uint32_t* goff = B.sgb_off + (size_t)(SGB_BUCKETS + 1) * g;
  for (uint32_t b = t; b <= SGB_BUCKETS; b += kSgbSortBlock) {
    goff[b] = off[b];
    if (b < SGB_BUCKETS) cnt[b] = off[b];
  }
  __syncthreads();
  uint32_t* ent = B.sgb_ent + (size_t)m * SGB_K * g;
  for (uint32_t li = t; li < n; li += kSgbSortBlock) {
#pragma unroll 1
    for (uint32_t k = 0; k < SGB_K; ++k) {
      const int32_t d = dig[li * SGB_K + k];
      if (!d) continue;
      const uint32_t pos = atomicAdd(&cnt[k * SGB_V + (uint32_t)(d < 0 ? -d : d) - 1], 1u);
      ent[pos] = (li << 1) | (d < 0 ? 1u : 0u);
    }
  }
}

__global__ void TBG_LAUNCH_N(TBG_PAIR_WAVES) k_sgb_bucket(DevBatch B, uint32_t n_sg) {
  const uint32_t w = (blockIdx.x * blockDim.x + threadIdx.x) >> 1;
  const uint32_t S = B.sgb_split, m = B.sgb_m;
  if (w >= n_sg * SGB_BUCKETS * S) return;
  const uint32_t g = w / (SGB_BUCKETS * S), b = (w / S) % SGB_BUCKETS, sl = w % S;
  const uint32_t* goff = B.sgb_off + (size_t)(SGB_BUCKETS + 1) * g;
  const uint32_t o0 = goff[b], n = goff[b + 1] - o0;
  const uint32_t e0 = o0 + (n * sl) / S, e1 = o0 + (n * (sl + 1)) / S;
  const uint32_t* ent = B.sgb_ent + (size_t)m * SGB_K * g;
  const G2A* sig = B.sig_aff + (size_t)m * g;
  Jac<Fp2x> acc = jac_inf<Fp2x>();
#pragma unroll 1
  for (uint32_t e = e0; e < e1; ++e) {
    const uint32_t v = ent[e];
    Aff<Fp2x> p = px_load(sig[v >> 1]);
    p.y = f_reduce(p.y);
    if (v & 1u) p.y = f_reduce(f_neg(p.y));
    acc = jac_add_aff_in(acc, p);
  }
  px_store(B.sgb_part[w], acc);
}

__global__ void TBG_LAUNCH_N(TBG_PAIR_WAVES) k_sgb_fold(DevBatch B, uint32_t n_sg) {
  const uint32_t w = (blockIdx.x * blockDim.x + threadIdx.x) >> 1;
  if (w >= n_sg * SGB_BUCKETS) return;
  const uint32_t S = B.sgb_split;
  G2J* part = B.sgb_part + (size_t)w * S;
  Jac<Fp2x> acc = px_load(part[0]);
  bool exc = false;
#pragma unroll 1
  for (uint32_t sl = 1; sl < S; ++sl) acc = jac_add_x(acc, px_load(part[sl]), exc);
  if (pair_all(!exc)) px_store(part[0], acc);
  else if (pair_par() == 0) B.sgb_bad[w / SGB_BUCKETS] = 1u;
}

__global__ void TBG_LAUNCH_N(TBG_PAIR_WAVES) k_sgb_combine(DevBatch B, uint32_t n_sg) {
  const uint32_t w = (blockIdx.x * blockDim.x + threadIdx.x) >> 1;
  if (w >= n_sg * SGB_K) return;
  const uint32_t g = w / SGB_K, k = w % SGB_K, S = B.sgb_split;
  G2J* part = B.sgb_part + ((size_t)SGB_BUCKETS * g + (size_t)SGB_V * k) * S;
  Jac<Fp2x> run = jac_inf<Fp2x>(), q = run;
  bool exc = false;
#pragma unroll 1
  for (int v = (int)SGB_V; v >= 1; --v) {
    run = jac_add_x(run, px_load(part[(size_t)(v - 1) * S]), exc);
    q = jac_add_x(q, run, exc);
  }
  if (pair_all(!exc)) px_store(part[0], q);
  else if (pair_par() == 0) B.sgb_bad[g] = 1u;
}

__global__ void TBG_LAUNCH_N(TBG_PAIR_WAVES) k_sgb_test(DevBatch B, uint32_t n_sg) {
  const uint32_t w = (blockIdx.x * blockDim.x + threadIdx.x) >> 1;
  if (w >= n_sg * SGB_K) return;
  const uint32_t g = w / SGB_K, k = w % SGB_K;
  const G2J& slot = B.sgb_part[((size_t)SGB_BUCKETS * g + (size_t)SGB_V * k) * B.sgb_split];
  bool ok = true;
  if (!jac_is_inf(px_load(slot))) {
    bool exc = false;
    Jac<Fp2x> m = px_load(slot);
#pragma unroll 1
    for (int i = 62; i >= 0; --i) {
      m = jac_dbl_lo(m);
      if ((X_ABS >> i) & 1) {
        __asm__ __volatile__("" ::: "memory");
        m = jac_add_x(m, px_load(slot), exc);
      }
    }
    if (exc || jac_is_inf(m)) {
      ok = false;
    } else {
      __asm__ __volatile__("" ::: "memory");
      const Jac<Fp2x> ps = g2_psi_g(px_load(slot));
      const Fp2x z1 = f_sqr(ps.Z), z2 = f_sqr(m.Z);
      ok = f_eq(f_mul(ps.X, z2), f_mul(m.X, z1)) &&
           f_eq(f_mul(f_mul(ps.Y, m.Z), z2), f_reduce(f_neg(f_mul(f_mul(m.Y, ps.Z), z1))));
    }
  }
  if (!ok && pair_par() == 0) B.sgb_bad[g] = 1u;
}

void launch_subgroup_batch(const DevBatch& B, hipStream_t st) {
  if (!B.sgb) return;
  const uint32_t n_sg = sgb_groups(B.n_partials, B.sgb_m);
  if (!n_sg) return;
  TBG_KLAUNCH(k_sgb_sort, dim3(n_sg), dim3(kSgbSortBlock), st, B);
  TBG_KLAUNCH(k_sgb_bucket, grid_for(2 * n_sg * SGB_BUCKETS * B.sgb_split), dim3(kBlock), st, B, n_sg);
  if (B.sgb_split > 1) TBG_KLAUNCH(k_sgb_fold, grid_for(2 * n_sg * SGB_BUCKETS), dim3(kBlock), st, B, n_sg);
  TBG_KLAUNCH(k_sgb_combine, grid_for(2 * n_sg * SGB_K), dim3(kBlock), st, B, n_sg);
  TBG_KLAUNCH(k_sgb_test, grid_for(2 * n_sg * SGB_K), dim3(kBlock), st, B, n_sg);
}

}
```

### charon_amd/csrc/tbls_engine.hip

```cpp
#include <hip/hip_runtime.h>
#include <cstdio>
#include <cstdlib>
#include <cstring>
#include <cmath>
#include <functional>
#include <algorithm>
#include <atomic>
#include <chrono>
#include <mutex>
#include <new>
#include <random>
#include <thread>
#include <vector>
#include "tbls_launch.h"
#include "bls_lines.h"

using namespace tbg;

namespace tbg {
void debug_after_launch(const char* kernel, hipStream_t st) {
  static const bool on = getenv("TBG_DEBUG_SYNC") && getenv("TBG_DEBUG_SYNC")[0] == '1';
  if (!on) return;
  hipEvent_t a;
  (void)hipEventCreate(&a);
// ... 251 lines not shown
  *out = c;
  return TBG_OK;
}

void tbg_destroy(tbg_ctx* c) {
  if (!c) return;
  hipSetDevice(c->device);
  if (c->stream) hipStreamSynchronize(c->stream);
  for (auto& s : c->slots) {
    if (s.st) hipStreamSynchronize(s.st);
    if (s.st2 && s.st2 != s.st) hipStreamSynchronize(s.st2);
    if (s.h_in) hipHostFree(s.h_in);
    if (s.h_out) hipHostFree(s.h_out);
    if (s.d_in) hipFree(s.d_in);
    if (s.d_work) hipFree(s.d_work);
    for (auto& e : s.ev)
      if (e) hipEventDestroy(e);
    if (s.done) hipEventDestroy(s.done);
    if (s.st2 && s.st2 != s.st) hipStreamDestroy(s.st2);
    if (s.st) hipStreamDestroy(s.st);
  }
  if (c->stream) {
    for (void* p : {(void*)c->d_pk, (void*)c->d_xpk, (void*)c->d_pktab, (void*)c->d_pk_status})
      if (p) hipFreeAsync(p, c->stream);
    hipStreamSynchronize(c->stream);
    hipStreamDestroy(c->stream);
  }
  if (c->retire_ev) hipEventDestroy(c->retire_ev);
  if (c->keys_ready) hipEventDestroy(c->keys_ready);
  delete c;
}

uint32_t tbg_pubkey_count(const tbg_ctx* c) { return c ? c->n_pk : 0; }

int tbg_load_pubkeys(tbg_ctx* c, const uint8_t* pk48, uint32_t count, uint32_t* first_id, int32_t* status) {
  if (!c || (count && !pk48)) return TBG_E_INVALID_ARG;
  std::lock_guard<std::mutex> lk(c->mu);
  HIP_TRY(hipSetDevice(c->device));
  if (c->n_pk + (uint64_t)count > 0xFFFFFFF0ull) return TBG_E_INVALID_ARG;
  uint32_t need = c->n_pk + count;
  void* old_tabs[4] = {nullptr, nullptr, nullptr, nullptr};
  if (need > c->cap_pk) {
    uint32_t ncap = need + need / 2 + 1024;
    G1A* npk = nullptr;
    G1A* nxpk = nullptr;
    G1A* ntab = nullptr;
    int32_t* nst = nullptr;
    hipStream_t us = c->stream;
    if (hipMallocAsync((void**)&npk, sizeof(G1A) * (size_t)ncap, us) != hipSuccess) return TBG_E_OOM;
    if (hipMallocAsync((void**)&nxpk, sizeof(G1A) * (size_t)ncap, us) != hipSuccess) {
      hipFreeAsync(npk, us);
      return TBG_E_OOM;
    }
    if (hipMallocAsync((void**)&ntab, PK_TAB * sizeof(G1A) * (size_t)ncap, us) != hipSuccess) {
      hipFreeAsync(npk, us);
      hipFreeAsync(nxpk, us);
      return TBG_E_OOM;
    }
    if (hipMallocAsync((void**)&nst, sizeof(int32_t) * (size_t)ncap, us) != hipSuccess) {
      hipFreeAsync(npk, us);
      hipFreeAsync(nxpk, us);
      hipFreeAsync(ntab, us);
      return TBG_E_OOM;
    }
    if (c->n_pk) {
      HIP_TRY(hipMemcpyAsync(npk, c->d_pk, sizeof(G1A) * (size_t)c->n_pk, hipMemcpyDeviceToDevice, us));
      HIP_TRY(hipMemcpyAsync(nxpk, c->d_xpk, sizeof(G1A) * (size_t)c->n_pk, hipMemcpyDeviceToDevice, us));
      HIP_TRY(hipMemcpyAsync(ntab, c->d_pktab, PK_TAB * sizeof(G1A) * (size_t)c->n_pk, hipMemcpyDeviceToDevice, us));
      HIP_TRY(hipMemcpyAsync(nst, c->d_pk_status, sizeof(int32_t) * (size_t)c->n_pk, hipMemcpyDeviceToDevice, us));
    }
    old_tabs[0] = c->d_pk;
    old_tabs[1] = c->d_xpk;
    old_tabs[2] = c->d_pktab;
    old_tabs[3] = c->d_pk_status;
    c->d_pk = npk;
    c->d_xpk = nxpk;
    c->d_pktab = ntab;
    c->d_pk_status = nst;
    c->cap_pk = ncap;
  }
  if (first_id) *first_id = c->n_pk;
  uint8_t* d_bytes = nullptr;
  if (count && hipMallocAsync((void**)&d_bytes, 48ull * count, c->stream) != hipSuccess) return TBG_E_OOM;
  int rc = TBG_OK;
  if (count == 0) goto ready;
  if (hipMemcpyAsync(d_bytes, pk48, 48ull * count, hipMemcpyHostToDevice, c->stream) != hipSuccess) rc = TBG_E_DEVICE;
  if (rc == TBG_OK) {
    launch_decode_pubkeys(d_bytes, count, c->d_pk + c->n_pk, c->d_xpk + c->n_pk, c->d_pk_status + c->n_pk, c->stream);
    launch_pubkey_tables(c->d_pk + c->n_pk, c->d_xpk + c->n_pk, c->d_pk_status + c->n_pk, count,
                         c->d_pktab + (size_t)PK_TAB * c->n_pk, c->stream);
    if (hipGetLastError() != hipSuccess) rc = TBG_E_DEVICE;
  }
  if (rc == TBG_OK && status &&
      hipMemcpyAsync(status, c->d_pk_status + c->n_pk, sizeof(int32_t) * count, hipMemcpyDeviceToHost, c->stream) != hipSuccess)
    rc = TBG_E_DEVICE;
ready:
  if (hipEventRecord(c->keys_ready, c->stream) != hipSuccess) rc = TBG_E_DEVICE;
  if (old_tabs[0]) {
    for (auto& sl : c->slots)
      for (hipStream_t q : {sl.st, sl.st2}) {
        if (!q || (q == sl.st2 && sl.st2 == sl.st)) continue;
        if (hipEventRecord(c->retire_ev, q) != hipSuccess || hipStreamWaitEvent(c->stream, c->retire_ev, 0) != hipSuccess)
          rc = TBG_E_DEVICE;
      }
    for (void* p : old_tabs) hipFreeAsync(p, c->stream);
  }
  if (d_bytes) hipFreeAsync(d_bytes, c->stream);
  if (hipEventSynchronize(c->keys_ready) != hipSuccess) rc = TBG_E_DEVICE;
  if (rc == TBG_OK) c->n_pk += count;
  return rc;
}

static void spec_aggregation(const DevBatch& B, hipStream_t st) {
  launch_lagrange(B, st, true);
  launch_aggregate(B, st, true);
  launch_aggregate_finish(B, st, true);
}

static int launch_chain(tbg_ctx* c, const Slot& sl, const DevBatch& B, hipEvent_t* ev, int stage = -1) {
  hipStream_t st = sl.st, st2 = sl.st2;
  const bool verify = B.op != TBG_OP_AGGREGATE;
  const G1A* pk = (const G1A*)c->d_pk;
  const bool spec = B.op == TBG_OP_VERIFY_AGGREGATE && (TBG_SPEC_ALWAYS || (B.rlc_batch && B.rlc_group));
  auto msg_chain = [&]() -> int {
    HIP_TRY(hipEventRecord(ev[3], st2));
    if (verify) launch_hash_msgs(B, st2);
    HIP_TRY(hipEventRecord(ev[4], st2));
    if (verify) launch_h_lines(B, st2);
    HIP_TRY(hipEventRecord(ev[5], st2));
    return TBG_OK;
  };
  auto sig_chain = [&]() -> int {
    HIP_TRY(hipEventRecord(ev[10], st));
    launch_decode_sigs(B, st);
    HIP_TRY(hipEventRecord(ev[1], st));
    if (verify)
      launch_rlc_prepare(B, pk, (const G1A*)c->d_xpk, (const G1A*)c->d_pktab, (const int32_t*)c->d_pk_status, c->n_pk,
                         st, spec ? spec_aggregation : nullptr);
    HIP_TRY(hipEventRecord(ev[2], st));
    return TBG_OK;
  };
  const bool alt = TBG_ALT_ORDER && st == st2 && ((&sl - c->slots.data()) & 1);
  int rc;
  if (stage < 0 || stage == 0) {
    HIP_TRY(hipEventRecord(ev[0], st));
    HIP_TRY(hipStreamWaitEvent(st2, ev[0], 0));
    if ((rc = alt ? sig_chain() : msg_chain()) != TBG_OK) return rc;
  }
  if (stage < 0 || stage == 1)
    if ((rc = alt ? msg_chain() : sig_chain()) != TBG_OK) return rc;
  if (stage >= 0 && stage != 2) return TBG_OK;
  HIP_TRY(hipStreamWaitEvent(st, ev[5], 0));
  HIP_TRY(hipEventRecord(ev[6], st));
  if (verify) launch_rlc_check(B, pk, (const G1A*)c->d_xpk, (const int32_t*)c->d_pk_status, c->n_pk, st);
  HIP_TRY(hipEventRecord(ev[7], st));
  if (B.op != TBG_OP_VERIFY) launch_lagrange(B, st);
  HIP_TRY(hipEventRecord(ev[8], st));
  launch_aggregate(B, st);
  if (B.op != TBG_OP_VERIFY) launch_aggregate_finish(B, st);
  HIP_TRY(hipEventRecord(ev[9], st));
  HIP_TRY(hipGetLastError());
  return TBG_OK;
}

static void chain_times(hipEvent_t* e, float* ms) {
  hipEventElapsedTime(&ms[0], e[10], e[1]);
  hipEventElapsedTime(&ms[1], e[3], e[4]);
  hipEventElapsedTime(&ms[2], e[1], e[2]);
  hipEventElapsedTime(&ms[3], e[4], e[5]);
  hipEventElapsedTime(&ms[4], e[6], e[7]);
  hipEventElapsedTime(&ms[5], e[7], e[8]);
  hipEventElapsedTime(&ms[6], e[8], e[9]);
  hipEventElapsedTime(&ms[7], e[0], e[9]);
}

static int validate(const tbg_batch* b) {
  if (!b) return TBG_E_INVALID_ARG;
  if (b->op < TBG_OP_VERIFY || b->op > TBG_OP_VERIFY_AGGREGATE) return TBG_E_INVALID_ARG;
  if (b->n_duties == 0) return TBG_E_INVALID_ARG;
  if (!b->duty_first || (b->n_partials && (!b->sigs || !b->identifiers))) return TBG_E_INVALID_ARG;
  if (b->duty_first[0] != 0 || b->duty_first[b->n_duties] != b->n_partials) return TBG_E_INVALID_ARG;
  for (uint32_t d = 0; d < b->n_duties; ++d) {
    if (b->duty_first[d + 1] < b->duty_first[d]) return TBG_E_INVALID_ARG;
    if (b->duty_first[d + 1] - b->duty_first[d] > 255) return TBG_E_INVALID_ARG;
  }
  if (b->op != TBG_OP_AGGREGATE) {
    if (!b->msg_off || !b->duty_msg || !b->pubkey_ids || b->n_msgs == 0) return TBG_E_INVALID_ARG;
    if (b->msg_off[0] != 0) return TBG_E_INVALID_ARG;
    for (uint32_t m = 0; m < b->n_msgs; ++m)
      if (b->msg_off[m + 1] < b->msg_off[m]) return TBG_E_INVALID_ARG;
    if (b->msg_off[b->n_msgs] && !b->msgs) return TBG_E_INVALID_ARG;
    for (uint32_t d = 0; d < b->n_duties; ++d)
      if (b->duty_msg[d] >= b->n_msgs) return TBG_E_INVALID_ARG;
  }
  if (b->op == TBG_OP_VERIFY_AGGREGATE && !b->duty_threshold) return TBG_E_INVALID_ARG;
  return TBG_OK;
}

static Slot* find_ticket(tbg_ctx* c, tbg_ticket t, bool want_pending, Part** part) {
  for (auto& x : c->slots)
    for (auto& q : x.parts)
      if (q.ticket == t && (want_pending ? q.pending : !x.busy)) {
        if (part) *part = &q;
        return &x;
      }
  return nullptr;
}

int tbg_submit(tbg_ctx* c, const tbg_batch* b, tbg_ticket* ticket) { return tbg_submit_group(c, &b, 1, ticket); }

static double l0_shape_cost(uint64_t nd, uint32_t n_simd, uint32_t g, uint32_t ch) {
  const uint64_t hexads = (uint64_t)((nd + g - 1) / g) * ((g + ch - 1) / ch);
  const uint64_t waves = (hexads + 9) / 10;
  return (0.948 + 1.395 * ch) * (double)((waves + n_simd - 1) / n_simd);
}
static bool l0_fits_any(uint32_t, uint32_t) { return true; }
static void l0_shape(uint64_t nd, uint32_t n_simd, bool g_free, uint32_t& G, uint32_t& C,
                     const std::function<bool(uint32_t, uint32_t)>& fits) {
  C = 4;
  if (!TBG_L0_SHAPE || G < 8) return;
  constexpr uint32_t L0_SHAPE_MAX_C = 10;
  uint32_t cand[3 + L0_SHAPE_MAX_C][2] = {{g_free ? 16u : G, 4}, {g_free ? 16u : G, 8}, {14, 7}};
  uint32_t n_cand = g_free ? 3u : 2u;
  for (uint32_t c = 5; TBG_L0_SHAPE_WIDE && g_free && c <= L0_SHAPE_MAX_C; ++c) {
    cand[n_cand][0] = c;
    cand[n_cand][1] = c;
    ++n_cand;
  }
  double best = 1e300;
  const uint32_t G0 = G;
  for (uint32_t k = 0; k < n_cand; ++k) {
    if (!fits(cand[k][0], cand[k][1])) continue;
    const double cost = l0_shape_cost(nd, n_simd, cand[k][0], cand[k][1]);
    if (cost < best - 1e-9) {
      best = cost;
      G = cand[k][0];
      C = cand[k][1];
    }
  }
  if (best == 1e300) G = G0;
}
static bool l0_shape_fits(uint32_t nd0, uint32_t G0, uint32_t C0, uint32_t nd, uint32_t G, uint32_t C) {
  const uint64_t ng0 = (nd0 + G0 - 1) / G0, nch0 = (G0 + C0 - 1) / C0;
  const uint64_t ng = (nd + G - 1) / G, nch = (G + C - 1) / C;
  return ng <= ng0 && ng * (nch + 1) <= ng0 * (nch0 + 1) && ng * nch <= ng0 * nch0 && ng * nch * C <= ng0 * nch0 * C0 &&
         ng * G <= ng0 * G0 && std::max(ng * nch, (uint64_t)nd) <= std::max(ng0 * nch0, (uint64_t)nd0) &&
         (G <= 64) == (G0 <= 64);
}

static bool sgb_plan(double rho, uint32_t& m) {
  double best = 1e9;
  m = SGB_M;
  for (uint32_t k = SGB_M; k >= SGB_M_MIN; k >>= 1) {
    const double cost = 0.55 + 1.1 * (double)SGB_K / k + (1.0 - std::pow(1.0 - std::min(rho, 1.0), (double)k));
    if (cost < best - 1e-12) {
      best = cost;
      m = k;
    }
  }
  return best < 0.95;
}

int tbg_submit_group(tbg_ctx* c, const tbg_batch* const* bs, uint32_t n_batches, tbg_ticket* tickets) {
  if (!c || !bs || !tickets || n_batches == 0) return TBG_E_INVALID_ARG;
  int rc;
  for (uint32_t k = 0; k < n_batches; ++k) {
    if ((rc = validate(bs[k])) != TBG_OK) return rc;
    if (bs[k]->op != bs[0]->op) return TBG_E_INVALID_ARG;
  }
  const uint32_t op = bs[0]->op;
  const bool verify = op != TBG_OP_AGGREGATE;
  uint64_t nd64 = 0, np64 = 0, nm64 = 0, mb64 = 0;
  for (uint32_t k = 0; k < n_batches; ++k) {
    nd64 += bs[k]->n_duties;
    np64 += bs[k]->n_partials;
    if (verify) {
      nm64 += bs[k]->n_msgs;
      mb64 += bs[k]->msg_off[bs[k]->n_msgs];
    }
  }
  if (np64 > 0x7FFFFFFFull || nd64 > 0x7FFFFFFFull || nm64 > 0x7FFFFFFFull || mb64 > 0xFFFFFFFFull)
    return TBG_E_INVALID_ARG;
  std::unique_lock<std::mutex> lk(c->mu);
  HIP_TRY(hipSetDevice(c->device));
  Slot* s = nullptr;
  const bool small = np64 <= c->express_max;
  for (auto& x : c->slots)
    if (x.express && small && !x.busy) s = &x;
  if (!s)
    for (auto& x : c->slots)
      if (!x.express && !x.busy && (!s || x.ticket < s->ticket)) s = &x;
  if (!s) return TBG_E_BUSY;

  const uint32_t nd = (uint32_t)nd64, np = (uint32_t)np64, nm = (uint32_t)nm64;
  const size_t msg_bytes = (size_t)mb64;

  size_t o = 0;
  auto sec = [&](size_t bytes) { size_t at = o; o = align_up(o + bytes, 16); return at; };
  size_t o_msgs = sec(msg_bytes);
  size_t o_msg_off = sec(4ull * (nm + 1));
  size_t o_duty_msg = sec(4ull * nd);
  size_t o_duty_first = sec(4ull * (nd + 1));
  size_t o_thr = sec(4ull * nd);
  size_t o_pduty = sec(4ull * np);
  size_t o_sigs = sec(96ull * np);
  size_t o_ids = sec(np);
  size_t o_pk = sec(4ull * np);
  size_t in_bytes = o;
  o = 0;
  size_t w_sig_aff = sec(sizeof(G2A) * (size_t)np);
  size_t w_h_aff = sec(sizeof(G2A) * (size_t)nm);
  size_t w_h_st = sec(4ull * nm);
  size_t w_h_jac = sec(3 * sizeof(G2J) * (size_t)nm);
  size_t w_lam = sec(32ull * np);
  const uint32_t fb_w = verify ? std::max<uint32_t>(1u, std::min<uint32_t>(c->fb_window, np)) : 0u;
  size_t w_sl = sec(4ull * LINES_WORDS * fb_w);
  size_t w_hl = sec(4ull * LINES_WORDS * nm);
  if (c->rlc_auto)
    c->rlc_group = c->invalid_ema < TBG_RLC_AUTO_TO8 ? 16 : c->invalid_ema < TBG_RLC_AUTO_TO4 ? 8 : 4;
  uint32_t G = verify ? c->rlc_group : 0;
  const bool l0 = G != 0 && np < (1u << 28) &&
                  (c->rlc_batch == TBG_RLC_L0_ON || (c->rlc_batch == TBG_RLC_L0_AUTO && c->invalid_ema < TBG_RLC_AUTO_L0));
  uint32_t C = c->rlc_chunk;
  if (l0 && c->chunk_auto) l0_shape(nd, c->n_simd, c->rlc_auto && G == 16, G, C, l0_fits_any);
  if (C > G) C = G ? G : 1;
  const uint32_t ng = G ? (nd + G - 1) / G : 0;
  const uint32_t nch = G ? (G + C - 1) / C : 0;
  size_t w_pp = sec(G ? sizeof(G1J) * (size_t)np : 0);
  size_t w_ps = sec(G ? sizeof(G2J) * (size_t)np : 0);
  size_t w_cf = sec(G ? 4ull * 3 * 4 * NL * ng * (nch + 1) : 0);
  size_t w_cl = sec(G > 1 ? 4ull * ng * nch : 0);

  size_t w_dvp = sec(G ? sizeof(G1A) * (size_t)nd : 0);
  size_t w_dvs = sec(G ? sizeof(G2J) * (size_t)nd : 0);
  size_t w_dvst = sec(G ? 4ull * nd : 0);
  size_t w_gst = sec(4ull * ng);
  size_t w_gl = sec(4ull * LINES_WORDS * ng);
  size_t w_cnt = sec(4ull * CNT_WORDS);
  size_t w_pl = sec(verify ? 4ull * np : 0);
  size_t w_dvfe = sec(G > 1 ? 4ull * 3 * 4 * NL * nd : 0);
  size_t w_pend = sec(G ? sizeof(G2A) * (size_t)std::max<size_t>(std::max<size_t>(ng, (size_t)ng * nch), nd) : 0);
  size_t w_cfe = sec(G > 1 ? 4ull * 3 * 4 * NL * ng * nch : 0);
  size_t w_cidl = sec(G > 1 ? 4ull * ng * nch : 0);
  size_t w_cidp = sec(G > 1 ? sizeof(G1A) * (size_t)ng * nch * C : 0);

  size_t w_gfe = sec(G > 1 ? 4ull * 3 * 4 * NL * ng : 0);
  size_t w_gidl = sec(G > 1 ? 4ull * ng : 0);
  size_t w_gidp = sec(G > 1 ? sizeof(G1A) * (size_t)ng * G : 0);
  size_t w_gidf = sec(G > 1 ? 4ull * 3 * 4 * NL * ng * (nch + 1) : 0);
  size_t w_idl = sec(G > 1 ? 4ull * nd : 0);
  size_t w_idp = sec(G > 1 ? sizeof(G1A) * (size_t)nd : 0);
  size_t w_mr = sec(l0 ? 8ull * np : 0);
  size_t w_moff = sec(l0 ? 4ull * (MSM_BUCKETS + 1) : 0);
  size_t w_mcur = sec(l0 ? 4ull * MSM_BUCKETS : 0);
  size_t w_ment = sec(l0 ? 16ull * np : 0);
  size_t w_mbkt = sec(l0 ? sizeof(G2J) * (size_t)MSM_BUCKETS : 0);
  size_t w_mpart = sec(l0 ? sizeof(G2J) * (size_t)MSM_BUCKETS * MSM_SPLIT : 0);
  size_t w_msum = sec(l0 ? sizeof(G2J) * (size_t)MSM_SUM_ENTRIES : 0);
  size_t w_bpt = sec(l0 ? sizeof(G2A) : 0);
  size_t w_blines = sec(l0 ? 4ull * LINES_WORDS : 0);
  size_t w_bf = sec(l0 ? 4ull * 3 * 4 * NL : 0);
  size_t w_gf = sec(l0 ? 4ull * 3 * 4 * NL * grp_f_entries(ng) : 0);
  const bool gm = TBG_GMSM && G != 0;
  size_t w_gmoff = sec(gm ? 4ull * (GM_BUCKETS + 1) * ng : 0);
  size_t w_gment = sec(gm ? 64ull * np : 0);
  size_t w_gmpart = sec(gm ? sizeof(G2J) * GM_BUCKETS * (size_t)ng : 0);
  size_t w_gmlead = sec(gm ? 4ull * ng : 0);
  size_t w_gmlist = sec(gm ? 4ull * np : 0);
  size_t w_gmhist = sec(gm ? 4ull * 256 : 0);
  size_t w_gmorder = sec(gm ? 4ull * GM_BUCKETS * ng : 0);
  uint32_t sgb_m = SGB_M;
  const bool sgb = np >= SGB_MIN_PARTIALS && c->sgb_mode != TBG_SGB_OFF &&
                   (sgb_plan(c->nonsub_ema, sgb_m) || c->sgb_mode == TBG_SGB_ON);
  const uint32_t sgb_split = sgb_split_for(sgb_m);
  const size_t n_sg = sgb ? sgb_groups(np, sgb_m) : 0;
  size_t w_sgoff = sec(4ull * (SGB_BUCKETS + 1) * n_sg);
  size_t w_sgent = sec(4ull * sgb_m * SGB_K * n_sg);
  size_t w_sgpart = sec(sizeof(G2J) * SGB_BUCKETS * sgb_split * n_sg);
  size_t w_sgbad = sec(4ull * n_sg);
  size_t w_aacc = sec(op != TBG_OP_VERIFY ? sizeof(G2J) * (size_t)nd : 0);
  size_t w_alist = sec(op != TBG_OP_VERIFY ? 4ull * nd : 0);
  size_t w_out = o;
  size_t w_pst = sec(4ull * np);
  size_t w_dst = sec(4ull * nd);
  size_t w_agg = sec(96ull * nd);
  size_t work_bytes = o;
  size_t out_bytes = work_bytes - w_out;

  if ((rc = grow_pinned(&s->h_in, &s->h_in_cap, in_bytes)) != TBG_OK) return rc;
  if ((rc = grow_pinned(&s->h_out, &s->h_out_cap, out_bytes)) != TBG_OK) return rc;
  if ((rc = grow_device(&s->d_in, &s->d_in_cap, in_bytes)) != TBG_OK) return rc;
  if ((rc = grow_device(&s->d_work, &s->d_work_cap, work_bytes)) != TBG_OK) return rc;
  s->parts.clear();
  s->busy = true;
  lk.unlock();
  const auto t_pack = std::chrono::steady_clock::now();

  uint8_t* h = s->h_in;
  uint32_t* msg_off = (uint32_t*)(h + o_msg_off);
  uint32_t* duty_msg = (uint32_t*)(h + o_duty_msg);
  uint32_t* duty_first = (uint32_t*)(h + o_duty_first);
  uint32_t* thr = (uint32_t*)(h + o_thr);
  uint32_t* pd = (uint32_t*)(h + o_pduty);
  std::vector<Part> parts(n_batches);
  std::vector<uint32_t> mb0(n_batches);
  uint32_t D = 0, P = 0, M = 0, MB = 0;
  for (uint32_t k = 0; k < n_batches; ++k) {
    const tbg_batch* b = bs[k];
    parts[k].d0 = D;
    parts[k].nd = b->n_duties;
    parts[k].p0 = P;
    parts[k].np = b->n_partials;
    parts[k].m0 = M;
    parts[k].nm = verify ? b->n_msgs : 0;
    mb0[k] = MB;
    D += parts[k].nd;
    P += parts[k].np;
    M += parts[k].nm;
    if (verify) MB += b->msg_off[b->n_msgs];
  }
  auto pack = [&](uint32_t k) {
    const tbg_batch* b = bs[k];
    const uint32_t D = parts[k].d0, P = parts[k].p0, M = parts[k].m0, MB = mb0[k];
    const uint32_t bnd = b->n_duties, bnp = b->n_partials, bnm = parts[k].nm;
    if (verify) {
      const uint32_t bmb = b->msg_off[bnm];
      if (bmb) memcpy(h + o_msgs + MB, b->msgs, bmb);
      for (uint32_t m = 0; m < bnm; ++m) msg_off[M + m] = MB + b->msg_off[m];
      for (uint32_t d = 0; d < bnd; ++d) duty_msg[D + d] = M + b->duty_msg[d];
      memcpy(h + o_pk + 4ull * P, b->pubkey_ids, 4ull * bnp);
    }
    for (uint32_t d = 0; d < bnd; ++d) {
      duty_first[D + d] = P + b->duty_first[d];
      for (uint32_t j = b->duty_first[d]; j < b->duty_first[d + 1]; ++j) pd[P + j] = D + d;
    }
    if (op == TBG_OP_VERIFY_AGGREGATE) memcpy(thr + D, b->duty_threshold, 4ull * bnd);
    else memset(thr + D, 0, 4ull * bnd);
    if (bnp) {
      memcpy(h + o_sigs + 96ull * P, b->sigs, 96ull * bnp);
      memcpy(h + o_ids + P, b->identifiers, bnp);
    }
  };
  const uint32_t workers = (np >= (1u << 16) && n_batches > 1) ? std::min<uint32_t>(n_batches, 8) : 1;
  if (workers == 1) {
    for (uint32_t k = 0; k < n_batches; ++k) pack(k);
  } else {
    std::vector<std::thread> th;
    for (uint32_t w = 0; w < workers; ++w)
      th.emplace_back([&, w] {
        for (uint32_t k = w; k < n_batches; k += workers) pack(k);
      });
    for (auto& t : th) t.join();
  }
  duty_first[nd] = np;
  if (verify) msg_off[nm] = MB;
  const auto t_packed = std::chrono::steady_clock::now();

  lk.lock();
  auto release = [&](int code) {
    s->busy = false;
    return code;
  };
  if (hipSetDevice(c->device) != hipSuccess) return release(TBG_E_DEVICE);
  DevBatch B{};
  memset(&B, 0, sizeof(B));
  B.op = op;
  B.n_duties = nd;
  B.n_partials = np;
  B.n_msgs = nm;
  uint8_t* di = s->d_in;
  uint8_t* dw = s->d_work;
  B.msgs = di + o_msgs;
  B.msg_off = (const uint32_t*)(di + o_msg_off);
  B.duty_msg = (const uint32_t*)(di + o_duty_msg);
  B.duty_first = (const uint32_t*)(di + o_duty_first);
  B.duty_threshold = (const uint32_t*)(di + o_thr);
  B.partial_duty = (const uint32_t*)(di + o_pduty);
  B.sigs = di + o_sigs;
  B.identifiers = di + o_ids;
  B.pubkey_ids = (const uint32_t*)(di + o_pk);
  B.sig_aff = (G2A*)(dw + w_sig_aff);
  B.h_aff = (G2A*)(dw + w_h_aff);
  B.h_status = (int32_t*)(dw + w_h_st);
  B.h_jac = (G2J*)(dw + w_h_jac);
  B.lam = (uint32_t*)(dw + w_lam);
  B.sig_lines = (uint32_t*)(dw + w_sl);
  B.h_lines = (uint32_t*)(dw + w_hl);
  B.rlc_group = G;
  {
    uint64_t k[4];
    if (c->rlc_seed) {
      uint64_t z = c->rlc_seed;
      for (auto& w : k) {
        z += 0x9E3779B97F4A7C15ull;
        uint64_t x = z;
        x = (x ^ (x >> 30)) * 0xBF58476D1CE4E5B9ull;
        x = (x ^ (x >> 27)) * 0x94D049BB133111EBull;
        w = x ^ (x >> 31);
      }
    } else {
      std::random_device rd;
      for (auto& w : k) w = ((uint64_t)rd() << 32) ^ rd() ^ (++c->seed_ctr * 0x9E3779B97F4A7C15ull);
    }
    for (int j = 0; j < 4; ++j) {
      B.rlc_seed[2 * j] = (uint32_t)(k[j] >> 32);
      B.rlc_seed[2 * j + 1] = (uint32_t)k[j];
    }
    std::random_device rd;
    for (auto& w : B.sgb_seed) w = rd() ^ (uint32_t)(++c->seed_ctr * 0x9E3779B9u);
  }
  B.rlc_chunk = C;
  B.part_p = (G1J*)(dw + w_pp);
  B.part_s = (G2J*)(dw + w_ps);
  B.chunk_f = (uint32_t*)(dw + w_cf);
  B.chunk_list = (uint32_t*)(dw + w_cl);
  B.chunk_lines = B.sig_lines;
  B.dv_p = (G1A*)(dw + w_dvp);
  B.dv_s = (G2J*)(dw + w_dvs);
  B.dv_state = (int32_t*)(dw + w_dvst);
  B.grp_state = (int32_t*)(dw + w_gst);
  B.grp_lines = (uint32_t*)(dw + w_gl);
  B.counters = (uint32_t*)(dw + w_cnt);
  B.part_list = (uint32_t*)(dw + w_pl);
  B.id_fe = (uint32_t*)(dw + w_dvfe);
  B.pend_pts = (G2A*)(dw + w_pend);
  B.chunk_fe = (uint32_t*)(dw + w_cfe);
  B.cid_list = (uint32_t*)(dw + w_cidl);
  B.cid_p = (G1A*)(dw + w_cidp);
  B.cid_lines = B.sig_lines;
  B.gident = G > 1 && G <= 64 ? c->gident : 0u;
  B.grp_fe = (uint32_t*)(dw + w_gfe);
  B.gid_list = (uint32_t*)(dw + w_gidl);
  B.gid_p = (G1A*)(dw + w_gidp);
  B.gid_lines = B.sig_lines;
  B.gid_f = (uint32_t*)(dw + w_gidf);
  B.id_list = (uint32_t*)(dw + w_idl);
  B.id_p = (G1A*)(dw + w_idp);
  B.id_lines = B.sig_lines;
  B.fb_window = fb_w;
  {
    const double share = std::min(1.0, 10.0 * c->invalid_ema);
    const uint64_t expect = (uint64_t)((double)np * share);
    B.fb_full = (!TBG_FB_EXPECT || G == 0 || fb_w == 0) ? 0xFFFFFFFFu
                                      : (uint32_t)std::min<uint64_t>(0xFFFFFFFFull, (expect / fb_w + 1) * (uint64_t)fb_w);
  }
  B.fb_base = 0;
  B.partial_status = (int32_t*)(dw + w_pst);
  B.duty_status = (int32_t*)(dw + w_dst);
  B.agg = dw + w_agg;
  B.rlc_batch = l0 ? 1u : 0u;
  B.msm_r = (uint64_t*)(dw + w_mr);
  B.msm_off = (uint32_t*)(dw + w_moff);
  B.msm_cur = (uint32_t*)(dw + w_mcur);
  B.msm_ent = (uint32_t*)(dw + w_ment);
  B.msm_bkt = (G2J*)(dw + w_mbkt);
  B.msm_part = (G2J*)(dw + w_mpart);
  B.msm_sum = (G2J*)(dw + w_msum);
  B.batch_pt = (G2A*)(dw + w_bpt);
  B.batch_lines = (uint32_t*)(dw + w_blines);
  B.batch_f = (uint32_t*)(dw + w_bf);
  B.grp_f = (uint32_t*)(dw + w_gf);
  B.gm_off = (uint32_t*)(dw + w_gmoff);
  B.gm_ent = (uint32_t*)(dw + w_gment);
  B.gm_part = (G2J*)(dw + w_gmpart);
  B.gm_lead = (uint32_t*)(dw + w_gmlead);
  B.gm_list = (uint32_t*)(dw + w_gmlist);
  B.gm_hist = (uint32_t*)(dw + w_gmhist);
  B.gm_order = (uint32_t*)(dw + w_gmorder);
  B.sgb = sgb ? 1u : 0u;
  B.sgb_m = sgb_m;
  B.sgb_split = sgb_split;
  B.sgb_off = (uint32_t*)(dw + w_sgoff);
  B.sgb_ent = (uint32_t*)(dw + w_sgent);
  B.sgb_part = (G2J*)(dw + w_sgpart);
  B.sgb_bad = (uint32_t*)(dw + w_sgbad);
  B.agg_acc = (G2J*)(dw + w_aacc);
  B.agg_list = (uint32_t*)(dw + w_alist);

  hipStream_t st = s->st;
  if (hipStreamWaitEvent(st, c->keys_ready, 0) != hipSuccess ||
      hipMemcpyAsync(s->d_in, s->h_in, in_bytes, hipMemcpyHostToDevice, st) != hipSuccess)
    return release(TBG_E_DEVICE);
  rc = launch_chain(c, *s, B, s->ev);
  if (rc != TBG_OK) return release(rc);
  if (hipMemcpyAsync(s->h_out, dw + w_out, out_bytes, hipMemcpyDeviceToHost, st) != hipSuccess ||
      hipEventRecord(s->done, st) != hipSuccess)
    return release(TBG_E_DEVICE);
  {
    const auto t_end = std::chrono::steady_clock::now();
    using ns = std::chrono::nanoseconds;
    c->host[0] += 1;
    c->host[1] += np;
    c->host[2] += (uint64_t)std::chrono::duration_cast<ns>(t_packed - t_pack).count();
    c->host[3] += (uint64_t)std::chrono::duration_cast<ns>(t_end - t_packed).count();
  }

  for (uint32_t k = 0; k < n_batches; ++k) {
    parts[k].ticket = c->next_ticket++;
    parts[k].pending = true;
    tickets[k] = parts[k].ticket;
  }
  s->parts = std::move(parts);
  s->seen_bad = s->seen_total = 0;
  s->seen_nsub = s->seen_dec = 0;
  s->busy = true;
  s->ticket = s->parts[0].ticket;
  s->op = op;
  s->n_duties = nd;
  s->n_partials = np;
  s->n_msgs = nm;
  s->out_bytes = out_bytes;
  s->B = B;
  s->last = B;
  s->w_out = w_out;
  return TBG_OK;
}

int tbg_poll(tbg_ctx* c, tbg_ticket t) {
  if (!c) return TBG_E_INVALID_ARG;
  std::lock_guard<std::mutex> lk(c->mu);
  Slot* s = find_ticket(c, t, true, nullptr);
  if (!s) return TBG_E_TICKET;
  HIP_TRY(hipSetDevice(c->device));
  hipError_t q = hipEventQuery(s->done);
  if (q == hipErrorNotReady) return TBG_E_PENDING;
  return q == hipSuccess ? TBG_OK : TBG_E_DEVICE;
}

static void copy_part(const Slot* s, const Part& q, int32_t* pst, int32_t* dst, uint8_t* agg) {
  const uint32_t np = s->n_partials, nd = s->n_duties;
  size_t o = 0;
  auto sec = [&](size_t bytes) { size_t at = o; o = align_up(o + bytes, 16); return at; };
  size_t o_pst = sec(4ull * np), o_dst = sec(4ull * nd), o_agg = sec(96ull * nd);
  if (pst) memcpy(pst, s->h_out + o_pst + 4ull * q.p0, 4ull * q.np);
  if (dst) memcpy(dst, s->h_out + o_dst + 4ull * q.d0, 4ull * q.nd);
  if (agg) memcpy(agg, s->h_out + o_agg + 96ull * q.d0, 96ull * q.nd);
}

static void part_done(Slot* s, Part* q) {
  q->pending = false;
  bool any = false;
  for (const auto& x : s->parts) any |= x.pending;
  s->busy = any;
}

int tbg_collect(tbg_ctx* c, tbg_ticket t, int32_t* pst, int32_t* dst, uint8_t* agg, int block) {
  if (!c) return TBG_E_INVALID_ARG;
  std::unique_lock<std::mutex> lk(c->mu);
  Part* q = nullptr;
  Slot* s = find_ticket(c, t, true, &q);
  if (!s || q->collecting) return TBG_E_TICKET;
  HIP_TRY(hipSetDevice(c->device));
  hipError_t e = hipEventQuery(s->done);
  if (e == hipErrorNotReady) {
    if (!block) return TBG_E_PENDING;
    q->collecting = true;
    hipEvent_t done = s->done;
    int dev = c->device;
    lk.unlock();
    const auto t_wait = std::chrono::steady_clock::now();
    (void)hipSetDevice(dev);
    e = hipEventSynchronize(done);
    c->host[7] += (uint64_t)std::chrono::duration_cast<std::chrono::nanoseconds>(std::chrono::steady_clock::now() -
                                                                                 t_wait).count();
    lk.lock();
    q->collecting = false;
  }
  if (e != hipSuccess) {
    part_done(s, q);
    return TBG_E_DEVICE;
  }
  const auto t_gather = std::chrono::steady_clock::now();
  copy_part(s, *q, pst, dst, agg);
  if (s->op != TBG_OP_AGGREGATE && q->np) {
    const int32_t* st = (const int32_t*)s->h_out;
    uint32_t bad = 0;
    for (uint32_t i = 0; i < q->np; ++i) bad += st[q->p0 + i] == TBG_PS_INVALID ? 1u : 0u;
    s->seen_bad += bad;
    s->seen_total += q->np;
  }
  if (q->np) {
    const int32_t* st = (const int32_t*)s->h_out;
    uint32_t ns = 0;
    for (uint32_t i = 0; i < q->np; ++i) ns += st[q->p0 + i] == TBG_PS_ERR_SUBGROUP ? 1u : 0u;
    s->seen_nsub += ns;
    s->seen_dec += q->np;
  }
  c->host[4] += 1;
  c->host[5] += q->np;
  c->host[6] += (uint64_t)std::chrono::duration_cast<std::chrono::nanoseconds>(std::chrono::steady_clock::now() -
                                                                               t_gather).count();
  chain_times(s->ev, s->ms);
  memcpy(c->last_ms, s->ms, sizeof(c->last_ms));
  part_done(s, q);
  if (!s->busy && s->seen_total) {
    c->invalid_ema = 0.5 * c->invalid_ema + 0.5 * (double)s->seen_bad / (double)s->seen_total;
    s->seen_bad = s->seen_total = 0;
  }
  if (!s->busy && s->seen_dec) {
    c->nonsub_ema = 0.5 * c->nonsub_ema + 0.5 * (double)s->seen_nsub / (double)s->seen_dec;
    s->seen_nsub = s->seen_dec = 0;
  }
  return TBG_OK;
}

int tbg_run(tbg_ctx* c, const tbg_batch* b, int32_t* pst, int32_t* dst, uint8_t* agg) {
  tbg_ticket t;
  int rc = tbg_submit(c, b, &t);
  if (rc != TBG_OK) return rc;
  return tbg_collect(c, t, pst, dst, agg, 1);
}

int tbg_replay_plan(tbg_ctx* c, const tbg_ticket* tickets, const uint32_t* n_parts, uint32_t n_launches, float* ms8) {
  if (!c || !tickets || n_launches == 0) return TBG_E_INVALID_ARG;
  std::lock_guard<std::mutex> lk(c->mu);
  std::vector<Slot*> sl(n_launches, nullptr);
  std::vector<DevBatch> bs(n_launches);
  for (uint32_t k = 0; k < n_launches; ++k) {
    sl[k] = find_ticket(c, tickets[k], false, nullptr);
    if (!sl[k]) return TBG_E_TICKET;
    DevBatch B = sl[k]->B;
    const uint32_t np = n_parts ? n_parts[k] : 0;
    if (np > sl[k]->parts.size()) return TBG_E_INVALID_ARG;
    if (np && np < sl[k]->parts.size()) {
      const Part& last = sl[k]->parts[np - 1];
      B.n_duties = last.d0 + last.nd;
      B.n_partials = last.p0 + last.np;
      B.n_msgs = last.m0 + last.nm;
// ... 357 lines not shown
    }
  }
  uint32_t n_chunks() const { return chunk_first.back(); }
  int upload(DevArena& a, const uint32_t* off, uint32_t n_sets, size_t part_elem, hipStream_t st, tbg::SumPlan& p) {
    uint32_t* d_off = (uint32_t*)a.sec(4ull * (n_sets + 1));
    uint32_t* d_cf = (uint32_t*)a.sec(4ull * (n_sets + 1));
    uint32_t* d_cs = (uint32_t*)a.sec(4ull * n_chunks() + 4);
    p.part = a.sec(part_elem * n_chunks() + 16);
    p.set_bad = (int32_t*)a.sec(4ull * n_sets + 4);
    p.n_sets = n_sets;
    p.n_chunks = n_chunks();
    p.off = d_off;
    p.chunk_first = d_cf;
    p.chunk_set = d_cs;
    if (hipMemcpyAsync(d_off, off, 4ull * (n_sets + 1), hipMemcpyHostToDevice, st) != hipSuccess ||
        hipMemcpyAsync(d_cf, chunk_first.data(), 4ull * (n_sets + 1), hipMemcpyHostToDevice, st) != hipSuccess ||
        (n_chunks() && hipMemcpyAsync(d_cs, chunk_set.data(), 4ull * n_chunks(), hipMemcpyHostToDevice, st) != hipSuccess) ||
        hipMemsetAsync(p.set_bad, 0, 4ull * n_sets, st) != hipSuccess)
      return TBG_E_DEVICE;
    return TBG_OK;
  }
};

}

extern "C" {

int tbg_sum_pubkeys(tbg_ctx* c, const uint32_t* pubkey_ids, const uint32_t* off, uint32_t n_sets, uint8_t* out48,
                    int32_t* status) {
  if (!c || !n_sets || !out48 || !status || !offsets_ok(off, n_sets)) return TBG_E_INVALID_ARG;
  const uint32_t ni = off[n_sets];
  if (ni && !pubkey_ids) return TBG_E_INVALID_ARG;
  std::lock_guard<std::mutex> lk(c->mu);
  HIP_TRY(hipSetDevice(c->device));
  SumHost h(off, n_sets);
  DevArena a;
  int rc = a.alloc(SumHost::bytes(n_sets, h.n_chunks(), sizeof(G1J)) + align_up(4ull * ni + 4, 16) +
                   align_up(48ull * n_sets, 16) + align_up(4ull * n_sets, 16));
  if (rc != TBG_OK) return rc;
  hipStream_t st = c->stream;
  tbg::SumPlan p;
  if ((rc = h.upload(a, off, n_sets, sizeof(G1J), st, p)) != TBG_OK) return rc;
  uint32_t* d_ids = (uint32_t*)a.sec(4ull * ni + 4);
  uint8_t* d_out = a.sec(48ull * n_sets);
  int32_t* d_st = (int32_t*)a.sec(4ull * n_sets);
  if (ni) HIP_TRY(hipMemcpyAsync(d_ids, pubkey_ids, 4ull * ni, hipMemcpyHostToDevice, st));
  tbg::launch_sum_g1(c->d_pk, c->d_pk_status, c->n_pk, d_ids, p, d_out, d_st, st);
  HIP_TRY(hipGetLastError());
  HIP_TRY(hipMemcpyAsync(out48, d_out, 48ull * n_sets, hipMemcpyDeviceToHost, st));
  HIP_TRY(hipMemcpyAsync(status, d_st, 4ull * n_sets, hipMemcpyDeviceToHost, st));
  HIP_TRY(hipStreamSynchronize(st));
  return TBG_OK;
}

int tbg_sum_sigs(tbg_ctx* c, const uint8_t* sigs96, const uint32_t* off, uint32_t n_sets, uint8_t* out96,
                 int32_t* status, int32_t* sig_status) {
  if (!c || !n_sets || !out96 || !status || !offsets_ok(off, n_sets)) return TBG_E_INVALID_ARG;
  const uint32_t ni = off[n_sets];
  if (ni && !sigs96) return TBG_E_INVALID_ARG;
  std::lock_guard<std::mutex> lk(c->mu);
  HIP_TRY(hipSetDevice(c->device));
  SumHost h(off, n_sets);
  DevArena a;
  int rc = a.alloc(SumHost::bytes(n_sets, h.n_chunks(), sizeof(G2J)) + align_up(96ull * ni + 4, 16) +
                   align_up(4ull * ni + 4, 16) + align_up(96ull * n_sets, 16) + align_up(4ull * n_sets, 16));
  if (rc != TBG_OK) return rc;
  hipStream_t st = c->stream;
  tbg::SumPlan p;
  if ((rc = h.upload(a, off, n_sets, sizeof(G2J), st, p)) != TBG_OK) return rc;
  uint8_t* d_sigs = a.sec(96ull * ni + 4);
  int32_t* d_sst = (int32_t*)a.sec(4ull * ni + 4);
  uint8_t* d_out = a.sec(96ull * n_sets);
  int32_t* d_st = (int32_t*)a.sec(4ull * n_sets);
  if (ni) HIP_TRY(hipMemcpyAsync(d_sigs, sigs96, 96ull * ni, hipMemcpyHostToDevice, st));
  tbg::launch_sum_g2(d_sigs, p, d_out, d_st, d_sst, st);
  HIP_TRY(hipGetLastError());
  HIP_TRY(hipMemcpyAsync(out96, d_out, 96ull * n_sets, hipMemcpyDeviceToHost, st));
  HIP_TRY(hipMemcpyAsync(status, d_st, 4ull * n_sets, hipMemcpyDeviceToHost, st));
  if (sig_status && ni) HIP_TRY(hipMemcpyAsync(sig_status, d_sst, 4ull * ni, hipMemcpyDeviceToHost, st));
  HIP_TRY(hipStreamSynchronize(st));
  return TBG_OK;
}

int tbg_fast_aggregate_verify(tbg_ctx* c, const uint32_t* pubkey_ids, const uint32_t* key_off, uint32_t n_sets,
                              const uint8_t* msgs, const uint32_t* msg_off, const uint8_t* sigs96, int32_t* status) {
  if (!c || !n_sets || !sigs96 || !status || !offsets_ok(key_off, n_sets) || !offsets_ok(msg_off, n_sets))
    return TBG_E_INVALID_ARG;
  const uint32_t nk = key_off[n_sets];
  const size_t mb = msg_off[n_sets];
  if ((nk && !pubkey_ids) || (mb && !msgs)) return TBG_E_INVALID_ARG;
  std::lock_guard<std::mutex> lk(c->mu);
  HIP_TRY(hipSetDevice(c->device));
  const uint32_t n = n_sets;
  SumHost h(key_off, n);
  std::vector<uint32_t> iota(n + 1);
  for (uint32_t i = 0; i <= n; ++i) iota[i] = i;
  const size_t lines = 4ull * LINES_WORDS * n;
  DevArena a;
  int rc = a.alloc(SumHost::bytes(n, h.n_chunks(), sizeof(G1J)) + align_up(4ull * nk + 4, 16) +
                   align_up(48ull * n, 16) * 2 + align_up(sizeof(G1A) * n, 16) * 2 + align_up(4ull * n, 16) * 6 +
                   align_up(mb + 1, 16) + align_up(4ull * (n + 1), 16) * 2 + align_up(96ull * n, 16) + align_up(n, 16) +
                   align_up(sizeof(G2A) * n, 16) * 2 + align_up(3 * sizeof(G2J) * n, 16) + 2 * align_up(lines, 16) +
                   align_up(4ull * tbg::CNT_WORDS, 16));
  if (rc != TBG_OK) return rc;
  hipStream_t st = c->stream;
  tbg::SumPlan p;
  if ((rc = h.upload(a, key_off, n, sizeof(G1J), st, p)) != TBG_OK) return rc;
  uint32_t* d_ids = (uint32_t*)a.sec(4ull * nk + 4);
  uint8_t* d_pk48 = a.sec(48ull * n);
  int32_t* d_kst = (int32_t*)a.sec(4ull * n);
  G1A* t_pk = (G1A*)a.sec(sizeof(G1A) * n);
  G1A* t_xpk = (G1A*)a.sec(sizeof(G1A) * n);
  int32_t* t_pkst = (int32_t*)a.sec(4ull * n);
  if (nk) HIP_TRY(hipMemcpyAsync(d_ids, pubkey_ids, 4ull * nk, hipMemcpyHostToDevice, st));
  tbg::launch_sum_g1(c->d_pk, c->d_pk_status, c->n_pk, d_ids, p, d_pk48, d_kst, st);
  tbg::launch_decode_pubkeys(d_pk48, n, t_pk, t_xpk, t_pkst, st);
  DevBatch B{};
  memset(&B, 0, sizeof(B));
  B.op = TBG_OP_VERIFY;
  B.n_duties = B.n_partials = B.n_msgs = n;
  uint8_t* d_msgs = a.sec(mb + 1);
  uint32_t* d_moff = (uint32_t*)a.sec(4ull * (n + 1));
  uint32_t* d_iota = (uint32_t*)a.sec(4ull * (n + 1));
  uint8_t* d_sigs = a.sec(96ull * n);
  uint8_t* d_idf = a.sec(n);
  B.msgs = d_msgs;
  B.msg_off = d_moff;
  B.duty_msg = B.duty_first = B.partial_duty = B.pubkey_ids = d_iota;
  B.duty_threshold = d_iota;
  B.sigs = d_sigs;
  B.identifiers = d_idf;
  B.sig_aff = (G2A*)a.sec(sizeof(G2A) * n);
  B.h_aff = (G2A*)a.sec(sizeof(G2A) * n);
  B.h_status = (int32_t*)a.sec(4ull * n);
  B.h_jac = (G2J*)a.sec(3 * sizeof(G2J) * n);
  B.sig_lines = (uint32_t*)a.sec(lines);
  B.h_lines = (uint32_t*)a.sec(lines);
  B.counters = (uint32_t*)a.sec(4ull * tbg::CNT_WORDS);
  B.part_list = (uint32_t*)a.sec(4ull * n);
  B.partial_status = (int32_t*)a.sec(4ull * n);
  B.duty_status = (int32_t*)a.sec(4ull * n);
  B.rlc_group = 0;
  B.fb_full = 0xFFFFFFFFu;
  if (mb) HIP_TRY(hipMemcpyAsync(d_msgs, msgs, mb, hipMemcpyHostToDevice, st));
  HIP_TRY(hipMemcpyAsync(d_moff, msg_off, 4ull * (n + 1), hipMemcpyHostToDevice, st));
  HIP_TRY(hipMemcpyAsync(d_iota, iota.data(), 4ull * (n + 1), hipMemcpyHostToDevice, st));
  HIP_TRY(hipMemcpyAsync(d_sigs, sigs96, 96ull * n, hipMemcpyHostToDevice, st));
  HIP_TRY(hipMemsetAsync(d_idf, 0, n, st));
  HIP_TRY(hipMemsetAsync(B.counters, 0, 4 * tbg::CNT_WORDS, st));
  tbg::launch_decode_sigs(B, st);
  tbg::launch_hash_msgs(B, st);
  tbg::launch_h_lines(B, st);
  tbg::launch_rlc_prepare(B, t_pk, t_xpk, nullptr, t_pkst, n, st);
  tbg::launch_rlc_check(B, t_pk, t_xpk, t_pkst, n, st);
  HIP_TRY(hipGetLastError());
  HIP_TRY(hipMemcpyAsync(status, B.partial_status, 4ull * n, hipMemcpyDeviceToHost, st));
  HIP_TRY(hipStreamSynchronize(st));
  return TBG_OK;
}

}
```

### charon_amd/csrc/tbls_launch.h

```cpp
#pragma once
#include <hip/hip_runtime.h>
#include "bls_curve.h"
#include "bls_lines.h"
#include "../../include/tbls_gpu.h"

namespace tbg {

constexpr int kBlock = 64;
#ifndef TBG_PK_W2
#define TBG_PK_W2 1
#endif
constexpr uint32_t PK_TAB = TBG_PK_W2 ? 8u : 2u;
#ifndef TBG_REPLAY_SHAPE
#define TBG_REPLAY_SHAPE 1
#endif
#ifndef TBG_L0_SHAPE
#define TBG_L0_SHAPE 1
#endif
#ifndef TBG_L0_SHAPE_WIDE
#define TBG_L0_SHAPE_WIDE 1
#endif
#ifndef TBG_FB_WINDOW
#define TBG_FB_WINDOW 32768u
#endif
#ifndef TBG_FB_EXPECT
#define TBG_FB_EXPECT 1
#endif

#ifndef TBG_MIN_WAVES
#define TBG_MIN_WAVES 1
#endif
#define TBG_LAUNCH __launch_bounds__(64, TBG_MIN_WAVES)
#ifndef TBG_PAIR_WAVES
#define TBG_PAIR_WAVES 2
#endif
#ifndef TBG_DECODE_WAVES
#define TBG_DECODE_WAVES 2
#endif
#define TBG_LAUNCH_N(w) __launch_bounds__(64, w)
#if defined(__HIP_DEVICE_COMPILE__)
#define TBG_URGENT() __builtin_amdgcn_s_setprio(3)
#else
#define TBG_URGENT() ((void)0)
#endif
inline dim3 grid_for(uint32_t n) { return dim3((n + kBlock - 1) / kBlock); }

struct DevBatch {
  uint32_t op, n_duties, n_partials, n_msgs;
  const uint8_t* msgs;
  const uint32_t* msg_off;
  const uint32_t* duty_msg;
  const uint32_t* duty_first;
  const uint32_t* duty_threshold;
  const uint32_t* partial_duty;
  const uint8_t* sigs;
  const uint8_t* identifiers;
  const uint32_t* pubkey_ids;
  G2A* sig_aff;
  G2A* h_aff;
  int32_t* h_status;
  G2J* h_jac;
  uint32_t* lam;
  uint32_t* sig_lines;
  uint32_t* h_lines;
  uint32_t rlc_seed[8];
  uint32_t rlc_group;
  G1J* part_p;
  G2J* part_s;
  uint32_t rlc_chunk;
  uint32_t* chunk_f;
  uint32_t* chunk_list;
  uint32_t* chunk_lines;
  G1A* dv_p;
  G2J* dv_s;
  int32_t* dv_state;
  int32_t* grp_state;
  uint32_t* grp_lines;
  uint32_t* counters;
  uint32_t* part_list;
  G2A* pend_pts;
  uint32_t* chunk_fe;
  uint32_t* cid_list;
  G1A* cid_p;
  uint32_t* cid_lines;
  uint32_t gident;
  uint32_t* grp_fe;
  uint32_t* gid_list;
  G1A* gid_p;
  uint32_t* gid_lines;
  uint32_t* gid_f;
  uint32_t* id_fe;
  uint32_t* id_list;
  G1A* id_p;
  uint32_t fb_window, fb_base;
  uint32_t fb_full;
  uint32_t* id_lines;
  uint32_t rlc_batch;
  uint64_t* msm_r;
  uint32_t* msm_off;
  uint32_t* msm_cur;
  uint32_t* msm_ent;
  G2J* msm_part;
  G2J* msm_bkt;
  G2J* msm_sum;
  G2A* batch_pt;
  uint32_t* batch_lines;
  uint32_t* batch_f;
  uint32_t* grp_f;
  uint32_t* gm_off;
  uint32_t* gm_ent;
  G2J* gm_part;
  uint32_t* gm_lead;
  uint32_t* gm_list;
  uint32_t* gm_hist;
  uint32_t* gm_order;
  uint32_t sgb;
  uint32_t sgb_m;
  uint32_t sgb_split;
  uint32_t sgb_seed[8];
  uint32_t* sgb_off;
  uint32_t* sgb_ent;
  G2J* sgb_part;
  uint32_t* sgb_bad;
  G2J* agg_acc;
  uint32_t* agg_list;
  int32_t* partial_status;
  int32_t* duty_status;
  uint8_t* agg;
};

enum RlcState : int32_t { RLC_NONE = 0, RLC_COMBINED = 1, RLC_EACH = 2 };
enum GroupState : int32_t { GRP_EMPTY = 0, GRP_LINES = 1, GRP_OK = 2, GRP_FAIL = 3, GRP_GID = 4 };
enum Counter : int { CNT_DUTIES = 0, CNT_PARTIALS = 1, CNT_AGG = 2, CNT_CHUNKS = 3, CNT_CID = 4, CNT_L0_BAD = 5,
                     CNT_L0_OK = 6, CNT_GID = 7, CNT_LAZY = 8, CNT_WORDS = 9 };

constexpr uint32_t MSM_BUCKETS = 32768;
constexpr uint32_t MSM_SPLIT = 4;
constexpr uint32_t MSM_SUM_ENTRIES = 128;
#ifndef TBG_SGB_M
#define TBG_SGB_M 1024
#endif
#ifndef TBG_SGB_SPLIT
#define TBG_SGB_SPLIT 4
#endif
constexpr uint32_t SGB_M = TBG_SGB_M;
constexpr uint32_t SGB_M_MIN = 64;
constexpr uint32_t SGB_K = 18;
constexpr uint32_t SGB_V = 6;
constexpr uint32_t SGB_BUCKETS = SGB_K * SGB_V;
constexpr uint32_t SGB_SPLIT = TBG_SGB_SPLIT;
constexpr uint32_t SGB_MIN_PARTIALS = 2 * SGB_M;
TBG_HD uint32_t sgb_groups(uint32_t n_partials, uint32_t m) { return (n_partials + m - 1) / m; }
TBG_HD uint32_t sgb_split_for(uint32_t m) {
  const uint32_t s = SGB_SPLIT * m / SGB_M;
  return s ? s : 1u;
}
constexpr uint32_t L0_TREE_FAN = 4;
TBG_HD uint32_t grp_f_entries(uint32_t n_groups) { return n_groups + n_groups / (L0_TREE_FAN - 1) + 40; }
enum MillerMode : int { MILLER_GROUPS = 0, MILLER_L0 = 1, MILLER_GROUP_S = 2 };
enum DutySumPhase : int { DSUM_BOTH = 0, DSUM_L0_P = 1, DSUM_FALLBACK_S = 2, DSUM_P = 3 };
#ifndef TBG_GMSM
#define TBG_GMSM 1
#endif
constexpr uint32_t GM_W = 4, GM_V = 8, GM_BUCKETS = GM_W * GM_V;

constexpr uint32_t CHUNK_DEGENERATE = 0x80000000u;
constexpr uint32_t ID_DEGENERATE = 0x80000000u;
enum FoldKind : int { FOLD_GROUPS = 0, FOLD_CHUNKS = 1, FOLD_CID = 2, FOLD_IDENT = 3, FOLD_GID = 5 };

TBG_HD bool fb_in_pass(const DevBatch& B, uint32_t k) { return B.fb_window == 0 || k - B.fb_base < B.fb_window; }
TBG_HD size_t fb_slot(const DevBatch& B, uint32_t k) { return (size_t)LINES_WORDS * (k - B.fb_base); }
template <class F>
TBG_HD void fb_pass_loop(const DevBatch& B, uint32_t first, uint32_t stride, uint32_t count, F&& body) {
  const uint32_t w = B.fb_window ? B.fb_window : 0xFFFFFFFFu;
  for (uint32_t s = first; s < w; s += stride) {
    const uint32_t k = B.fb_base + s;
    if (k >= count) break;
    body(k);
  }
}

#ifndef TBG_SPEC_ALWAYS
#define TBG_SPEC_ALWAYS 0
#endif
#ifndef TBG_ALT_ORDER
#define TBG_ALT_ORDER 0
#endif
#ifndef TBG_L0_JOIN
#define TBG_L0_JOIN 0
#endif
template <bool SPEC = false>
TBG_HD bool participates(uint32_t op, int32_t st) {
  return op == TBG_OP_VERIFY_AGGREGATE ? (st == TBG_PS_VALID || (SPEC && st == TBG_PS_NOT_VERIFIED))
                                       : (st == TBG_PS_NOT_VERIFIED);
}

void debug_after_launch(const char* kernel, hipStream_t st);
void kprof_pre(const char* kernel, hipStream_t st);
void kprof_post(hipStream_t st);
#define TBG_KLAUNCH(kernel, grid, block, st, ...)                      \
  do {                                                                \
    kprof_pre(#kernel, st);                                           \
    hipLaunchKernelGGL(kernel, grid, block, 0, st, __VA_ARGS__);      \
    kprof_post(st);                                                   \
    debug_after_launch(#kernel, st);                                  \
  } while (0)

struct SumPlan {
  uint32_t n_sets, n_chunks;
  const uint32_t* off;
  const uint32_t* chunk_first;
  const uint32_t* chunk_set;
  void* part;
  int32_t* set_bad;
};
uint32_t sum_chunk_size();
void launch_sum_g1(const G1A* table, const int32_t* pk_status, uint32_t n_pk, const uint32_t* ids, const SumPlan& p,
                   uint8_t* out48, int32_t* status, hipStream_t st);
void launch_sum_g2(const uint8_t* sigs96, const SumPlan& p, uint8_t* out96, int32_t* status, int32_t* sig_status,
                   hipStream_t st);
void launch_decode_pubkeys(const uint8_t* pk48, uint32_t n, G1A* out, G1A* out_x, int32_t* status, hipStream_t st);
void launch_decode_sigs(const DevBatch& B, hipStream_t st);
void launch_subgroup_batch(const DevBatch& B, hipStream_t st);
void launch_hash_msgs(const DevBatch& B, hipStream_t st);
void launch_hash_clear(const DevBatch& B, hipStream_t st);
void launch_h_lines(const DevBatch& B, hipStream_t st);
void launch_rlc_prepare(const DevBatch& B, const G1A* pk_aff, const G1A* xpk_aff, const G1A* pk_tab,
                        const int32_t* pk_status, uint32_t n_pk, hipStream_t st,
                        void (*after_keys)(const DevBatch&, hipStream_t) = nullptr);
void launch_rlc_check(const DevBatch& B, const G1A* pk_aff, const G1A* xpk_aff, const int32_t* pk_status, uint32_t n_pk,
                      hipStream_t st);
void launch_lines_fold(const DevBatch& B, int kind, uint32_t max_entries, hipStream_t st);
void launch_pubkey_tables(const G1A* pk, const G1A* xpk, const int32_t* status, uint32_t n, G1A* tab, hipStream_t st);
void launch_l0_keys(const DevBatch& B, const G1A* pk_tab, const int32_t* pk_status, uint32_t n_pk, hipStream_t st);
void launch_l0_msm(const DevBatch& B, hipStream_t st);
void launch_l0_check(const DevBatch& B, hipStream_t st);
void launch_l0_miller_hex(const DevBatch& B, hipStream_t st);
void launch_groups_miller_hex(const DevBatch& B, hipStream_t st);
void launch_group_s_miller_hex(const DevBatch& B, hipStream_t st);
void launch_rlc_partials(const DevBatch& B, const G1A* pk_tab, const G1A* pk_aff, const int32_t* pk_status,
                         uint32_t n_pk, hipStream_t st);
void launch_rlc_g1(const DevBatch& B, const G1A* pk_tab, const G1A* pk_aff, const int32_t* pk_status, uint32_t n_pk,
                   hipStream_t st);
void launch_gm_group_s(const DevBatch& B, hipStream_t st);
void launch_gm_failed_partials(const DevBatch& B, const G1A* pk_aff, hipStream_t st);
void launch_rlc_partials_list(const DevBatch& B, const G1A* pk_aff, hipStream_t st);
void launch_lagrange(const DevBatch& B, hipStream_t st, bool spec = false);
void launch_aggregate(const DevBatch& B, hipStream_t st, bool spec = false);
void launch_aggregate_finish(const DevBatch& B, hipStream_t st, bool spec = false);
void launch_sk_to_pk(const uint8_t* sk32, uint32_t n, uint8_t* pk48, hipStream_t st);
void launch_sign(const uint8_t* sk32, const uint32_t* item_msg, uint32_t n, const G2A* h_aff, const int32_t* h_status,
                 uint8_t* sig96, hipStream_t st);

}
```

Measured before the change: 3.333 million DV-duties/s (n verifies + 1 aggregate each).

## Fuse level-0 batch G2 MSM with subgroup-check bucket sums via shared digits

When subgroup batching and level-0 RLC are both enabled, the level-0 random scalars are derived from the subgroup-check base-13 digits. The level-0 signature sum can then be rebuilt from the subgroup bucket partials plus small per-slice totals, using Horner steps and psi twists, instead of running a separate G2 MSM with its own bucket sort. Per-partial G1 key scalars use the same digits through a windowed table multiply. The fallback path now reruns the non-batched G1 keys and group sums when level 0 fails. This removes the separate MSM passes and their buffers, but it couples the randomness of the two checks and adds extra reduce, fold and Horner kernels plus more fallback work.

```diff
diff --git a/charon_amd/csrc/bls_pair.h b/charon_amd/csrc/bls_pair.h
--- a/charon_amd/csrc/bls_pair.h
+++ b/charon_amd/csrc/bls_pair.h
@@ -54,6 +54,19 @@
 template <class F>
 TBG_HD Jac<F> g2_psi_g(const Jac<F>& p) {
   return {f_mulc(f_conj(p.X), PSI_X), f_mulc(f_conj(p.Y), PSI_Y), f_reduce(f_conj(p.Z))};
+}
+
+template <class F>
+TBG_HD Jac<F> l0f_mul13_add(const Jac<F>& acc, const Jac<F>& q) {
+  Jac<F> t = jac_add_in<F, true>(jac_dbl_in(acc), acc);
+  t = jac_add_in<F, true>(jac_dbl_in(jac_dbl_in(t)), acc);
+  return jac_add_in<F, true>(t, q);
+}
+template <class F>
+TBG_HD Jac<F> l0f_term(const Jac<F>& A, const Jac<F>& T, int j) {
+  Jac<F> r = jac_add_in<F, true>(jac_dbl_in(A), T);
+  for (int k = 0; k < j; ++k) r = g2_psi_g(r);
+  return r;
 }
 
 template <class F>
diff --git a/charon_amd/csrc/bls_rlc.h b/charon_amd/csrc/bls_rlc.h
--- a/charon_amd/csrc/bls_rlc.h
+++ b/charon_amd/csrc/bls_rlc.h
@@ -131,6 +131,39 @@
   return acc;
 }
 
+TBG_HD int l0f_first(int j) { return j < 2 ? 5 * j : 10 + 4 * (j - 2); }
+TBG_HD int l0f_bits(int j) { return j < 2 ? 20 : 16; }
+TBG_HD void l0f_rho(const int32_t (&c)[18], int32_t (&rho)[4]) {
+  for (int j = 0; j < 4; ++j) {
+    int32_t v = 0;
+    for (int e = l0f_first(j + 1) - 1; e >= l0f_first(j); --e) v = 13 * v + c[e];
+    rho[j] = v;
+  }
+}
+TBG_HD void l0f_scalar(const int32_t (&c)[18], int32_t (&a)[4]) {
+  int32_t rho[4];
+  l0f_rho(c, rho);
+  for (int j = 0; j < 4; ++j) a[j] = 2 * rho[j] + 1;
+}
+TBG_HD void l0f_digits(const int32_t (&c)[18], uint32_t (&u)[4]) {
+  int32_t rho[4];
+  l0f_rho(c, rho);
+  for (int j = 0; j < 4; ++j) u[j] = (uint32_t)(rho[j] + (1 << (l0f_bits(j) - 1)));
+}
+template <class F>
+TBG_HD Jac<F> rlc_mul_key_l0f(const Aff<F>* tab, const Fp& c, const uint32_t (&u)[4]) {
+  Jac<F> acc = jac_from_aff(rlc_entry_w2(tab, rlc_win2(u[0], 9), rlc_win2(u[1], 9), false, c));
+  acc = jac_dbl_in(jac_dbl_in(acc));
+  acc = jac_add_aff_in(acc, rlc_entry_w2(tab, rlc_win2(u[0], 8), rlc_win2(u[1], 8), false, c));
+#pragma unroll 1
+  for (int i = 7; i >= 0; --i) {
+    acc = jac_dbl_in(jac_dbl_in(acc));
+    acc = jac_add_aff_in(acc, rlc_entry_w2(tab, rlc_win2(u[0], i), rlc_win2(u[1], i), false, c));
+    acc = jac_add_aff_in(acc, rlc_entry_w2(tab, rlc_win2(u[2], i), rlc_win2(u[3], i), true, c));
+  }
+  return acc;
+}
+
 #if defined(TBG_PK_W2)
 TBG_HD G1J rlc_mul_key(const G1A* tab, const uint32_t (&u)[4]) {
 #if TBG_PK_W2
diff --git a/charon_amd/csrc/k_decode.hip b/charon_amd/csrc/k_decode.hip
--- a/charon_amd/csrc/k_decode.hip
+++ b/charon_amd/csrc/k_decode.hip
@@ -38,7 +38,7 @@
 __global__ void TBG_LAUNCH_N(TBG_DECODE_WAVES) k_decode_sigs(DevBatch B) {
   uint32_t i = blockIdx.x * blockDim.x + threadIdx.x;
   if (i < CNT_WORDS) B.counters[i] = 0;
-  if (B.rlc_batch && i <= MSM_BUCKETS) B.msm_off[i] = 0;
+  if (B.rlc_batch && !l0_fused(B) && i <= MSM_BUCKETS) B.msm_off[i] = 0;
   if (i >= B.n_partials) return;
   G2A& a = B.sig_aff[i];
   int32_t st = g2_decompress_t<true, false>(B.sigs + 96ull * i, a, SlotKeep{&a.y});
@@ -73,7 +73,7 @@
 }
 void launch_decode_sigs(const DevBatch& B, hipStream_t st) {
   uint32_t lanes = B.n_partials > CNT_WORDS ? B.n_partials : CNT_WORDS;
-  if (B.rlc_batch && lanes < MSM_BUCKETS + 1) lanes = MSM_BUCKETS + 1;
+  if (B.rlc_batch && !l0_fused(B) && lanes < MSM_BUCKETS + 1) lanes = MSM_BUCKETS + 1;
   TBG_KLAUNCH(k_decode_sigs, grid_for(lanes), dim3(kBlock), st, B);
   launch_subgroup_batch(B, st);
   if (B.n_partials) TBG_KLAUNCH(k_subgroup_sigs, grid_for(2 * B.n_partials), dim3(kBlock), st, B);
diff --git a/charon_amd/csrc/k_gmsm.hip b/charon_amd/csrc/k_gmsm.hip
--- a/charon_amd/csrc/k_gmsm.hip
+++ b/charon_amd/csrc/k_gmsm.hip
@@ -24,6 +24,7 @@
 
 __global__ void TBG_LAUNCH k_rlc_g1(DevBatch B, const G1A* tab, const G1A* pk_aff, const int32_t* pk_status,
                                    uint32_t n_pk) {
+  if (B.counters[CNT_L0_OK]) return;
   const uint32_t i = blockIdx.x * blockDim.x + threadIdx.x;
   if (i >= B.n_partials || B.partial_status[i] != TBG_PS_NOT_VERIFIED) return;
   const uint32_t pid = B.pubkey_ids[i];
diff --git a/charon_amd/csrc/k_miller_hex.hip b/charon_amd/csrc/k_miller_hex.hip
--- a/charon_amd/csrc/k_miller_hex.hip
+++ b/charon_amd/csrc/k_miller_hex.hip
@@ -134,7 +134,8 @@
   const uint32_t np_q = MODE == MILLER_GROUP_S ? 0u : n_groups * nch;
   const uint32_t qd = hex_slot(t);
   if (qd == 0xFFFFFFFFu || qd >= np_q + (MODE == MILLER_L0 ? 1u : n_groups)) return;
-  if (MODE == MILLER_GROUP_S && B.counters[CNT_L0_OK]) return;
+  if (MODE != MILLER_L0 && B.counters[CNT_L0_OK]) return;
+  if (MODE == MILLER_L0 && l0_fused(B) && B.counters[CNT_L0_BAD]) return;
   const bool s_quad = qd >= np_q;
   const uint32_t* ls = nullptr;
   uint32_t* dst;
diff --git a/charon_amd/csrc/k_msm.hip b/charon_amd/csrc/k_msm.hip
--- a/charon_amd/csrc/k_msm.hip
+++ b/charon_amd/csrc/k_msm.hip
@@ -41,8 +41,16 @@
   const uint32_t i = blockIdx.x * blockDim.x + threadIdx.x;
   if (i >= B.n_partials || B.partial_status[i] != TBG_PS_NOT_VERIFIED) return;
   const uint32_t pid = B.pubkey_ids[i];
+  const bool fused = l0_fused(B);
   if (pid >= n_pk || pk_status[pid] != DEC_OK) {
     B.partial_status[i] = TBG_PS_ERR_PUBKEY;
+    if (fused) B.counters[CNT_L0_BAD] = 1;
+    return;
+  }
+  if (fused) {
+    const uint4 v = *(const uint4*)(B.l0f_u + 4ull * i);
+    const uint32_t uf[4] = {v.x, v.y, v.z, v.w};
+    B.part_p[i] = rlc_mul_key_l0f(tab + (size_t)PK_TAB * pid, fp_from_const(G1_BETA), uf);
     return;
   }
   const uint64_t r = rlc_scalar(B.rlc_seed, i);
@@ -230,6 +238,63 @@
   px_store(*B.batch_pt, Aff<Fp2x>{f_mul(acc.X, zi2), f_mul(acc.Y, f_mul(zi2, zi))});
 }
 
+__global__ void __launch_bounds__(2 * L0F_PAIRS) k_l0f_reduce(DevBatch B, uint32_t n_sg, uint32_t wq, uint32_t n_t) {
+  __shared__ Jac<Fp2x> lds[2 * L0F_PAIRS];
+  if (B.counters[CNT_L0_BAD]) return;
+  const uint32_t pr = threadIdx.x >> 1, b = blockIdx.x;
+  const bool qcol = b < SGB_K * wq;
+  const uint32_t col = qcol ? b / wq : SGB_K, chunk = qcol ? b % wq : b - SGB_K * wq;
+  const uint32_t count = qcol ? n_sg : n_sg * n_t;
+  const uint32_t a0 = chunk * L0F_CHUNK + pr * L0F_PER, a1 = min(a0 + L0F_PER, count);
+  Jac<Fp2x> acc = jac_inf<Fp2x>();
+#pragma unroll 1
+  for (uint32_t a = a0; a < a1; ++a) {
+    if (qcol) {
+      acc = jac_add_in<Fp2x, true>(acc, px_load(B.sgb_part[((size_t)SGB_BUCKETS * a + (size_t)SGB_V * col) * B.sgb_split]));
+    } else {
+      acc = jac_add_in<Fp2x, true>(acc, px_load(B.sgb_t[a]));
+    }
+  }
+  acc = pair_tree_sum<L0F_PAIRS>(acc, lds);
+  if (pr == 0) px_store(B.l0f_sum[b], acc);
+}
+
+__global__ void __launch_bounds__(2 * L0F_PAIRS) k_l0f_fold(DevBatch B, uint32_t wq, uint32_t wt) {
+  TBG_URGENT();
+  __shared__ Jac<Fp2x> lds[2 * L0F_PAIRS];
+  if (B.counters[CNT_L0_BAD]) return;
+  const uint32_t pr = threadIdx.x >> 1, col = blockIdx.x;
+  const uint32_t first = col < SGB_K ? col * wq : SGB_K * wq, count = col < SGB_K ? wq : wt;
+  Jac<Fp2x> acc = jac_inf<Fp2x>();
+#pragma unroll 1
+  for (uint32_t a = pr; a < count; a += L0F_PAIRS) acc = jac_add_in<Fp2x, true>(acc, px_load(B.l0f_sum[first + a]));
+  acc = pair_tree_sum<L0F_PAIRS>(acc, lds);
+  if (pr == 0) px_store(B.l0f_sum[SGB_K * wq + wt + col], acc);
+}
+
+constexpr uint32_t L0F_HORNER_THREADS = 8;
+__global__ void __launch_bounds__(64) k_l0f_horner(DevBatch B, uint32_t base) {
+  TBG_URGENT();
+  __shared__ Jac<Fp2x> lds[L0F_HORNER_THREADS];
+  if (B.counters[CNT_L0_BAD]) return;
+  const int j = (int)(threadIdx.x >> 1);
+  const G2J* tot = B.l0f_sum + base;
+  const int e0 = l0f_first(j), e1 = l0f_first(j + 1);
+  Jac<Fp2x> acc = px_load(tot[e1 - 1]);
+#pragma unroll 1
+  for (int e = e1 - 2; e >= e0; --e) acc = l0f_mul13_add(acc, px_load(tot[e]));
+  acc = l0f_term(acc, px_load(tot[SGB_K]), j);
+  acc = pair_tree_sum<L0F_HORNER_THREADS / 2>(acc, lds);
+  if (j != 0) return;
+  if (jac_is_inf(acc)) {
+    if (pair_par() == 0) B.counters[CNT_L0_BAD] = 1;
+    return;
+  }
+  const Fp2x zi = f_inv(acc.Z);
+  const Fp2x zi2 = f_sqr(zi);
+  px_store(*B.batch_pt, Aff<Fp2x>{f_mul(acc.X, zi2), f_mul(acc.Y, f_mul(zi2, zi))});
+}
+
 void launch_pubkey_tables(const G1A* pk, const G1A* xpk, const int32_t* status, uint32_t n, G1A* tab, hipStream_t st) {
   if (n) TBG_KLAUNCH(k_pubkey_tables, dim3((n + BINV_BLOCK - 1) / BINV_BLOCK), dim3(BINV_BLOCK), st, pk, xpk, status, n,
                      tab);
@@ -248,4 +313,12 @@
   TBG_KLAUNCH(k_msm_tree_final, dim3(1), dim3(MSM_TREE_WG), st, B);
 }
 
-}
+void launch_l0_fused_s(const DevBatch& B, hipStream_t st) {
+  const uint32_t n_sg = sgb_groups(B.n_partials, B.sgb_m), n_t = sgb_t_slices(B.sgb_m);
+  const uint32_t wq = l0f_q_chunks(n_sg), wt = l0f_t_chunks(n_sg, B.sgb_m);
+  TBG_KLAUNCH(k_l0f_reduce, dim3(SGB_K * wq + wt), dim3(2 * L0F_PAIRS), st, B, n_sg, wq, n_t);
+  TBG_KLAUNCH(k_l0f_fold, dim3(L0F_COLS), dim3(2 * L0F_PAIRS), st, B, wq, wt);
+  TBG_KLAUNCH(k_l0f_horner, dim3(1), dim3(L0F_HORNER_THREADS), st, B, SGB_K * wq + wt);
+}
+
+}
diff --git a/charon_amd/csrc/k_rlc.hip b/charon_amd/csrc/k_rlc.hip
--- a/charon_amd/csrc/k_rlc.hip
+++ b/charon_amd/csrc/k_rlc.hip
@@ -37,6 +37,7 @@
   constexpr int phase = PHASE;
   const uint32_t d = blockIdx.x * blockDim.x + threadIdx.x;
   const bool in = d < B.n_duties;
+  if (phase == DSUM_P && B.counters[CNT_L0_OK]) return;
   if (phase == DSUM_FALLBACK_S) {
     if (!in || B.counters[CNT_L0_OK] || B.dv_state[d] != RLC_COMBINED) return;
 #if TBG_GMSM
@@ -733,7 +734,8 @@
   if (B.rlc_batch) {
     launch_l0_keys(B, pk_tab, pk_status, n_pk, st);
     if (after_keys) after_keys(B, st);
-    launch_l0_msm(B, st);
+    if (l0_fused(B)) launch_l0_fused_s(B, st);
+    else launch_l0_msm(B, st);
     TBG_KLAUNCH(k_rlc_duty_sum<DSUM_L0_P>, duty_grid(B), dim3(BINV_BLOCK), st, B);
     launch_l0_lines(B, st);
     return;
@@ -751,9 +753,10 @@
   launch_lines_fold(B, FOLD_GROUPS, n_groups, st);
 }
 
-void launch_rlc_check(const DevBatch& B, const G1A* pk_aff, const G1A* xpk_aff, const int32_t* pk_status, uint32_t n_pk,
-                      hipStream_t st) {
-  if (!B.n_duties) return;
+void launch_rlc_check(const DevBatch& B0, const G1A* pk_aff, const G1A* xpk_aff, const G1A* pk_tab,
+                      const int32_t* pk_status, uint32_t n_pk, hipStream_t st) {
+  if (!B0.n_duties) return;
+  DevBatch B = B0;
   if (B.rlc_group != 0) {
     uint32_t n_groups = (B.n_duties + B.rlc_group - 1) / B.rlc_group;
     uint32_t nch = (B.rlc_group + B.rlc_chunk - 1) / B.rlc_chunk;
@@ -770,6 +773,14 @@
       }
       launch_l0_final(B, in, n, st);
       TBG_KLAUNCH(k_l0_after, grid_for(n_groups), dim3(kBlock), st, B);
+      if (l0_fused(B)) {
+        B.rlc_batch = 0;
+        launch_rlc_g1(B, pk_tab, pk_aff, pk_status, n_pk, st);
+        TBG_KLAUNCH(k_rlc_duty_sum<DSUM_P>, duty_grid(B), dim3(BINV_BLOCK), st, B);
+        launch_gm_group_s(B, st);
+        launch_lines_fold(B, FOLD_GROUPS, n_groups, st);
+        launch_groups_miller_hex(B, st);
+      } else {
 #if TBG_GMSM
       launch_gm_group_s(B, st);
 #else
@@ -779,6 +790,7 @@
 #endif
       launch_lines_fold(B, FOLD_GROUPS, n_groups, st);
       launch_group_s_miller_hex(B, st);
+      }
     } else {
       launch_groups_miller_hex(B, st);
     }
diff --git a/charon_amd/csrc/k_sgb.hip b/charon_amd/csrc/k_sgb.hip
--- a/charon_amd/csrc/k_sgb.hip
+++ b/charon_amd/csrc/k_sgb.hip
@@ -22,11 +22,17 @@
   const uint32_t n = min(m, B.n_partials - i0);
   for (uint32_t b = t; b < SGB_BUCKETS; b += kSgbSortBlock) cnt[b] = 0;
   if (t == 0) B.sgb_bad[g] = 0;
+  const bool fused = l0_fused(B);
   __syncthreads();
   for (uint32_t li = t; li < n; li += kSgbSortBlock) {
     const bool ok = B.partial_status[i0 + li] == TBG_PS_NOT_VERIFIED;
     int32_t c[SGB_K];
     sgb_digits(B.sgb_seed, i0 + li, c);
+    if (fused) {
+      uint32_t u[4];
+      l0f_digits(c, u);
+      *(uint4*)(B.l0f_u + 4ull * (i0 + li)) = make_uint4(u[0], u[1], u[2], u[3]);
+    }
 #pragma unroll
     for (uint32_t k = 0; k < SGB_K; ++k) {
       const int32_t d = ok ? c[k] : 0;
@@ -62,10 +68,25 @@
   }
 }
 
-__global__ void TBG_LAUNCH_N(TBG_PAIR_WAVES) k_sgb_bucket(DevBatch B, uint32_t n_sg) {
+__global__ void TBG_LAUNCH_N(TBG_PAIR_WAVES) k_sgb_bucket(DevBatch B, uint32_t n_sg, uint32_t n_t) {
   const uint32_t w = (blockIdx.x * blockDim.x + threadIdx.x) >> 1;
   const uint32_t S = B.sgb_split, m = B.sgb_m;
-  if (w >= n_sg * SGB_BUCKETS * S) return;
+  if (w >= n_sg * SGB_BUCKETS * S) {
+    const uint32_t wt = w - n_sg * SGB_BUCKETS * S;
+    if (wt >= n_sg * n_t) return;
+    const uint32_t i0 = (wt / n_t) * m + (wt % n_t) * SGB_T_PER;
+    const uint32_t i1 = min(min(i0 + SGB_T_PER, (wt / n_t + 1) * m), B.n_partials);
+    Jac<Fp2x> acc = jac_inf<Fp2x>();
+#pragma unroll 1
+    for (uint32_t i = i0; i < i1; ++i) {
+      if (B.partial_status[i] != TBG_PS_NOT_VERIFIED) continue;
+      Aff<Fp2x> p = px_load(B.sig_aff[i]);
+      p.y = f_reduce(p.y);
+      acc = jac_add_aff_in(acc, p);
+    }
+    px_store(B.sgb_t[wt], acc);
+    return;
+  }
   const uint32_t g = w / (SGB_BUCKETS * S), b = (w / S) % SGB_BUCKETS, sl = w % S;
   const uint32_t* goff = B.sgb_off + (size_t)(SGB_BUCKETS + 1) * g;
   const uint32_t o0 = goff[b], n = goff[b + 1] - o0;
@@ -84,6 +105,11 @@
   px_store(B.sgb_part[w], acc);
 }
 
+__device__ __forceinline__ void sgb_fail(const DevBatch& B, uint32_t g) {
+  B.sgb_bad[g] = 1u;
+  if (l0_fused(B)) B.counters[CNT_L0_BAD] = 1u;
+}
+
 __global__ void TBG_LAUNCH_N(TBG_PAIR_WAVES) k_sgb_fold(DevBatch B, uint32_t n_sg) {
   const uint32_t w = (blockIdx.x * blockDim.x + threadIdx.x) >> 1;
   if (w >= n_sg * SGB_BUCKETS) return;
@@ -94,7 +120,7 @@
 #pragma unroll 1
   for (uint32_t sl = 1; sl < S; ++sl) acc = jac_add_x(acc, px_load(part[sl]), exc);
   if (pair_all(!exc)) px_store(part[0], acc);
-  else if (pair_par() == 0) B.sgb_bad[w / SGB_BUCKETS] = 1u;
+  else if (pair_par() == 0) sgb_fail(B, w / SGB_BUCKETS);
 }
 
 __global__ void TBG_LAUNCH_N(TBG_PAIR_WAVES) k_sgb_combine(DevBatch B, uint32_t n_sg) {
@@ -110,7 +136,7 @@
     q = jac_add_x(q, run, exc);
   }
   if (pair_all(!exc)) px_store(part[0], q);
-  else if (pair_par() == 0) B.sgb_bad[g] = 1u;
+  else if (pair_par() == 0) sgb_fail(B, g);
 }
 
 __global__ void TBG_LAUNCH_N(TBG_PAIR_WAVES) k_sgb_test(DevBatch B, uint32_t n_sg) {
@@ -140,7 +166,7 @@
            f_eq(f_mul(f_mul(ps.Y, m.Z), z2), f_reduce(f_neg(f_mul(f_mul(m.Y, ps.Z), z1))));
     }
   }
-  if (!ok && pair_par() == 0) B.sgb_bad[g] = 1u;
+  if (!ok && pair_par() == 0) sgb_fail(B, g);
 }
 
 void launch_subgroup_batch(const DevBatch& B, hipStream_t st) {
@@ -148,7 +174,8 @@
   const uint32_t n_sg = sgb_groups(B.n_partials, B.sgb_m);
   if (!n_sg) return;
   TBG_KLAUNCH(k_sgb_sort, dim3(n_sg), dim3(kSgbSortBlock), st, B);
-  TBG_KLAUNCH(k_sgb_bucket, grid_for(2 * n_sg * SGB_BUCKETS * B.sgb_split), dim3(kBlock), st, B, n_sg);
+  const uint32_t n_t = l0_fused(B) ? sgb_t_slices(B.sgb_m) : 0u;
+  TBG_KLAUNCH(k_sgb_bucket, grid_for(2 * n_sg * (SGB_BUCKETS * B.sgb_split + n_t)), dim3(kBlock), st, B, n_sg, n_t);
   if (B.sgb_split > 1) TBG_KLAUNCH(k_sgb_fold, grid_for(2 * n_sg * SGB_BUCKETS), dim3(kBlock), st, B, n_sg);
   TBG_KLAUNCH(k_sgb_combine, grid_for(2 * n_sg * SGB_K), dim3(kBlock), st, B, n_sg);
   TBG_KLAUNCH(k_sgb_test, grid_for(2 * n_sg * SGB_K), dim3(kBlock), st, B, n_sg);
diff --git a/charon_amd/csrc/tbls_engine.hip b/charon_amd/csrc/tbls_engine.hip
--- a/charon_amd/csrc/tbls_engine.hip
+++ b/charon_amd/csrc/tbls_engine.hip
@@ -427,7 +427,8 @@
   if (stage >= 0 && stage != 2) return TBG_OK;
   HIP_TRY(hipStreamWaitEvent(st, ev[5], 0));
   HIP_TRY(hipEventRecord(ev[6], st));
-  if (verify) launch_rlc_check(B, pk, (const G1A*)c->d_xpk, (const int32_t*)c->d_pk_status, c->n_pk, st);
+  if (verify) launch_rlc_check(B, pk, (const G1A*)c->d_xpk, (const G1A*)c->d_pktab, (const int32_t*)c->d_pk_status,
+                                 c->n_pk, st);
   HIP_TRY(hipEventRecord(ev[7], st));
   if (B.op != TBG_OP_VERIFY) launch_lagrange(B, st);
   HIP_TRY(hipEventRecord(ev[8], st));
@@ -625,13 +626,6 @@
   size_t w_gidf = sec(G > 1 ? 4ull * 3 * 4 * NL * ng * (nch + 1) : 0);
   size_t w_idl = sec(G > 1 ? 4ull * nd : 0);
   size_t w_idp = sec(G > 1 ? sizeof(G1A) * (size_t)nd : 0);
-  size_t w_mr = sec(l0 ? 8ull * np : 0);
-  size_t w_moff = sec(l0 ? 4ull * (MSM_BUCKETS + 1) : 0);
-  size_t w_mcur = sec(l0 ? 4ull * MSM_BUCKETS : 0);
-  size_t w_ment = sec(l0 ? 16ull * np : 0);
-  size_t w_mbkt = sec(l0 ? sizeof(G2J) * (size_t)MSM_BUCKETS : 0);
-  size_t w_mpart = sec(l0 ? sizeof(G2J) * (size_t)MSM_BUCKETS * MSM_SPLIT : 0);
-  size_t w_msum = sec(l0 ? sizeof(G2J) * (size_t)MSM_SUM_ENTRIES : 0);
   size_t w_bpt = sec(l0 ? sizeof(G2A) : 0);
   size_t w_blines = sec(l0 ? 4ull * LINES_WORDS : 0);
   size_t w_bf = sec(l0 ? 4ull * 3 * 4 * NL : 0);
@@ -653,6 +647,18 @@
   size_t w_sgent = sec(4ull * sgb_m * SGB_K * n_sg);
   size_t w_sgpart = sec(sizeof(G2J) * SGB_BUCKETS * sgb_split * n_sg);
   size_t w_sgbad = sec(4ull * n_sg);
+  const bool fused = l0 && sgb && TBG_PK_W2;
+  const bool msm = l0 && !fused;
+  size_t w_mr = sec(msm ? 8ull * np : 0);
+  size_t w_moff = sec(msm ? 4ull * (MSM_BUCKETS + 1) : 0);
+  size_t w_mcur = sec(msm ? 4ull * MSM_BUCKETS : 0);
+  size_t w_ment = sec(msm ? 16ull * np : 0);
+  size_t w_mbkt = sec(msm ? sizeof(G2J) * (size_t)MSM_BUCKETS : 0);
+  size_t w_mpart = sec(msm ? sizeof(G2J) * (size_t)MSM_BUCKETS * MSM_SPLIT : 0);
+  size_t w_msum = sec(msm ? sizeof(G2J) * (size_t)MSM_SUM_ENTRIES : 0);
+  size_t w_sgt = sec(fused ? sizeof(G2J) * sgb_t_slices(sgb_m) * n_sg : 0);
+  size_t w_l0fsum = sec(fused ? sizeof(G2J) * (size_t)l0f_sum_entries((uint32_t)n_sg, sgb_m) : 0);
+  size_t w_l0fu = sec(fused ? 16ull * np : 0);
   size_t w_aacc = sec(op != TBG_OP_VERIFY ? sizeof(G2J) * (size_t)nd : 0);
   size_t w_alist = sec(op != TBG_OP_VERIFY ? 4ull * nd : 0);
   size_t w_out = o;
@@ -849,6 +855,9 @@
   B.sgb_ent = (uint32_t*)(dw + w_sgent);
   B.sgb_part = (G2J*)(dw + w_sgpart);
   B.sgb_bad = (uint32_t*)(dw + w_sgbad);
+  B.sgb_t = (G2J*)(dw + w_sgt);
+  B.l0f_sum = (G2J*)(dw + w_l0fsum);
+  B.l0f_u = (uint32_t*)(dw + w_l0fu);
   B.agg_acc = (G2J*)(dw + w_aacc);
   B.agg_list = (uint32_t*)(dw + w_alist);
 
@@ -1512,7 +1521,7 @@
   tbg::launch_hash_msgs(B, st);
   tbg::launch_h_lines(B, st);
   tbg::launch_rlc_prepare(B, t_pk, t_xpk, nullptr, t_pkst, n, st);
-  tbg::launch_rlc_check(B, t_pk, t_xpk, t_pkst, n, st);
+  tbg::launch_rlc_check(B, t_pk, t_xpk, nullptr, t_pkst, n, st);
   HIP_TRY(hipGetLastError());
   HIP_TRY(hipMemcpyAsync(status, B.partial_status, 4ull * n, hipMemcpyDeviceToHost, st));
   HIP_TRY(hipStreamSynchronize(st));
diff --git a/charon_amd/csrc/tbls_launch.h b/charon_amd/csrc/tbls_launch.h
--- a/charon_amd/csrc/tbls_launch.h
+++ b/charon_amd/csrc/tbls_launch.h
@@ -122,6 +122,9 @@
   uint32_t* sgb_ent;
   G2J* sgb_part;
   uint32_t* sgb_bad;
+  G2J* sgb_t;
+  G2J* l0f_sum;
+  uint32_t* l0f_u;
   G2J* agg_acc;
   uint32_t* agg_list;
   int32_t* partial_status;
@@ -154,6 +157,19 @@
 TBG_HD uint32_t sgb_split_for(uint32_t m) {
   const uint32_t s = SGB_SPLIT * m / SGB_M;
   return s ? s : 1u;
+}
+TBG_HD bool l0_fused(const DevBatch& B) {
+  return TBG_PK_W2 && B.rlc_batch && B.rlc_group && B.sgb && B.n_partials;
+}
+constexpr uint32_t SGB_T_PER = 32;
+TBG_HD uint32_t sgb_t_slices(uint32_t m) { return m / SGB_T_PER; }
+constexpr uint32_t L0F_COLS = SGB_K + 1;
+constexpr uint32_t L0F_PAIRS = 128, L0F_PER = 4;
+constexpr uint32_t L0F_CHUNK = L0F_PAIRS * L0F_PER;
+TBG_HD uint32_t l0f_q_chunks(uint32_t n_sg) { return (n_sg + L0F_CHUNK - 1) / L0F_CHUNK; }
+TBG_HD uint32_t l0f_t_chunks(uint32_t n_sg, uint32_t m) { return (n_sg * sgb_t_slices(m) + L0F_CHUNK - 1) / L0F_CHUNK; }
+TBG_HD uint32_t l0f_sum_entries(uint32_t n_sg, uint32_t m) {
+  return SGB_K * l0f_q_chunks(n_sg) + l0f_t_chunks(n_sg, m) + L0F_COLS;
 }
 constexpr uint32_t L0_TREE_FAN = 4;
 TBG_HD uint32_t grp_f_entries(uint32_t n_groups) { return n_groups + n_groups / (L0_TREE_FAN - 1) + 40; }
@@ -228,12 +244,13 @@
 void launch_rlc_prepare(const DevBatch& B, const G1A* pk_aff, const G1A* xpk_aff, const G1A* pk_tab,
                         const int32_t* pk_status, uint32_t n_pk, hipStream_t st,
                         void (*after_keys)(const DevBatch&, hipStream_t) = nullptr);
-void launch_rlc_check(const DevBatch& B, const G1A* pk_aff, const G1A* xpk_aff, const int32_t* pk_status, uint32_t n_pk,
-                      hipStream_t st);
+void launch_rlc_check(const DevBatch& B, const G1A* pk_aff, const G1A* xpk_aff, const G1A* pk_tab,
+                      const int32_t* pk_status, uint32_t n_pk, hipStream_t st);
 void launch_lines_fold(const DevBatch& B, int kind, uint32_t max_entries, hipStream_t st);
 void launch_pubkey_tables(const G1A* pk, const G1A* xpk, const int32_t* status, uint32_t n, G1A* tab, hipStream_t st);
 void launch_l0_keys(const DevBatch& B, const G1A* pk_tab, const int32_t* pk_status, uint32_t n_pk, hipStream_t st);
 void launch_l0_msm(const DevBatch& B, hipStream_t st);
+void launch_l0_fused_s(const DevBatch& B, hipStream_t st);
 void launch_l0_check(const DevBatch& B, hipStream_t st);
 void launch_l0_miller_hex(const DevBatch& B, hipStream_t st);
 void launch_groups_miller_hex(const DevBatch& B, hipStream_t st);
```

Result: faster. 3.410 million DV-duties/s (n verifies + 1 aggregate each), median of 6 (+2.3%).
